# eBay/Sequence-Semantic-Embedding

Hardware: AMD Instinct MI355X
Metric: encoded seqs/sec (+ query x target cosine-scores/sec, top-1 vs ref) (higher is better)
Workload: dtype f32; 1 GPU; configs[1]: classification stand-in, dual-encoder LSTM H=S=256 E=50 T=32 V=32000; encode 16384 source seqs/GPU/step + cosine top-10 vs 571-target index; batch_per_gpu=16384, seq_len=32, targets=571, parallelism=dp1, weights=random-init (reference initialisers, seed 0)

## Files before the change

sequence-semantic-embedding_amd/csrc/score_topk.hip:

```cpp
#include <cstdlib>

#include "sse_kernels.h"

#define SC_THREADS 512
#define SC_KC 16
#ifndef SC_PRIO_K
#define SC_PRIO_K 1
#define SC_PRIO_E 0
#endif

#ifdef SSE_SCORE_CLOCK
#include <cstdio>
__device__ long long g_score_clk[8 * 8];
#define SC_CLK_DECL long long ck_[8] = {0, 0, 0, 0, 0, 0, 0, 0}, ck_t = clock64();
#define SC_CLK(i)                   \
  {                                 \
    const long long n_ = clock64(); \
    ck_[i] += n_ - ck_t;            \
    ck_t = n_;                      \
  }
#else
#define SC_CLK_DECL
#define SC_CLK(i)
#endif
// ... 671 lines not shown
                NQ, (int)BF, a.KG, w, v[w * 8 + 4], v[w * 8 + 0] / t, v[w * 8 + 1] / t, v[w * 8 + 2] / t, v[w * 8 + 5] / t, v[w * 8 + 6] / t, v[w * 8 + 7] / t,
                (v[w * 8 + 0] + v[w * 8 + 1] + v[w * 8 + 2] + v[w * 8 + 5] + v[w * 8 + 6]) / t);
      }
    }
  }
#endif
  return hipGetLastError();
}

template <int NQ, bool BF, bool COLLECT>
static hipError_t launch_score_variant(const ScoreArgs &a, hipStream_t stream) {
  return (a.KG % 8 == 0) ? launch_score_ringed<NQ, BF, COLLECT, true>(a, stream) : launch_score_ringed<NQ, BF, COLLECT, false>(a, stream);
}

__global__ void compact_uncert_kernel(const int32_t *cert, int Q, int32_t *qmap, int32_t *count) {
  const int q = blockIdx.x * blockDim.x + threadIdx.x;
  const bool open_q = q < Q && cert[q] == 0;
  const unsigned long long m = __ballot(open_q);
  if (m == 0ull) return;
  const int lane = threadIdx.x & 63;
  int base = 0;
  if (lane == __ffsll((long long)m) - 1) base = atomicAdd(count, __popcll(m));
  base = __shfl(base, __ffsll((long long)m) - 1);
  if (open_q) qmap[base + __popcll(m & ((1ull << lane) - 1ull))] = q;
}
__global__ void gather_query_rows_kernel(const float *q, const int32_t *qmap, const int32_t *count, int Q, int S, float *qc) {
  const int slot = blockIdx.x * (blockDim.x >> 6) + (threadIdx.x >> 6), lane = threadIdx.x & 63;
  const int n = *count, padded = min(Q, (n + 31) & ~31);
  if (slot >= padded) return;
  const float *src = slot < n ? q + (size_t)qmap[slot] * S : nullptr;
  for (int d = lane; d < S; d += 64) qc[(size_t)slot * S + d] = src ? src[d] : 0.0f;
}
hipError_t launch_compact_uncert(const float *q, const int32_t *cert, int Q, int S, int32_t *qmap, int32_t *count, float *qc,
                                 hipStream_t st) {
  hipError_t e = hipMemsetAsync(count, 0, sizeof(int32_t), st);
  if (e != hipSuccess) return e;
  hipLaunchKernelGGL(compact_uncert_kernel, dim3((Q + 255) / 256), dim3(256), 0, st, cert, Q, qmap, count);
  hipLaunchKernelGGL(gather_query_rows_kernel, dim3((Q + 3) / 4), dim3(256), 0, st, q, qmap, count, Q, S, qc);
  return hipGetLastError();
}

__global__ void count_uncert_kernel(const int32_t *cert, int Q, unsigned long long *count) {
  const int q = blockIdx.x * blockDim.x + threadIdx.x;
  const unsigned long long m = __ballot(q < Q && cert[q] == 0);
  if ((threadIdx.x & 63) == 0 && m) atomicAdd(count, (unsigned long long)__popcll(m));
}
hipError_t launch_count_uncert(const int32_t *cert, int Q, unsigned long long *count, hipStream_t st) {
  hipLaunchKernelGGL(count_uncert_kernel, dim3((Q + 255) / 256), dim3(256), 0, st, cert, Q, count);
  return hipGetLastError();
}

__global__ void pack_rows_bf16_kernel(const float *__restrict__ rows, int64_t R, int C, int KG16, int64_t total8,
                                      f32x4 *__restrict__ out) {
  for (int64_t i = (int64_t)blockIdx.x * blockDim.x + threadIdx.x; i < total8; i += (int64_t)gridDim.x * blockDim.x) {
    const int l = (int)(i & 63);
    const int64_t blk = i >> 6;
    const int kg = (int)(blk % KG16);
    const int64_t r = (blk / KG16) * 32 + (l & 31);
    const int k0 = kg * 16 + (l >> 5) * 8;
    unsigned w[4] = {0, 0, 0, 0};
    if (r < R) {
      const float *src = rows + (size_t)r * C + k0;
#pragma unroll
      for (int j = 0; j < 8; ++j) {
        unsigned short b = 0;
        if (k0 + j < C) {
          unsigned u = __float_as_uint(src[j]);
          u += 0x7FFFu + ((u >> 16) & 1u);
          b = (unsigned short)(u >> 16);
        }
        w[j >> 1] |= (unsigned)b << ((j & 1) * 16);
      }
    }
    out[i] = __builtin_bit_cast(f32x4, u32x4{w[0], w[1], w[2], w[3]});
  }
}

hipError_t launch_pack_rows_bf16(const float *rows, int64_t R, int C, void *out, hipStream_t stream) {
  const int KG16 = (C + 15) / 16;
  const int64_t total8 = ((R + 31) / 32) * KG16 * 64;
  if (total8 == 0) return hipSuccess;
  const int64_t blocks = (total8 + 255) / 256;
  hipLaunchKernelGGL(pack_rows_bf16_kernel, dim3((int)(blocks < 16384 ? blocks : 16384)), dim3(256), 0, stream, rows, R, C, KG16,
                     total8, reinterpret_cast<f32x4 *>(out));
  return hipGetLastError();
}

__global__ void frag32_to_bf16_kernel(const f32x4 *__restrict__ in, int64_t NT, int KG, int KG16, int64_t total8,
                                      f32x4 *__restrict__ out) {
  for (int64_t i = (int64_t)blockIdx.x * blockDim.x + threadIdx.x; i < total8; i += (int64_t)gridDim.x * blockDim.x) {
    const int l = (int)(i & 63);
    const int64_t blk = i >> 6;
    const int kg16 = (int)(blk % KG16);
    const int64_t tile = blk / KG16;
    const int kg = kg16 * 2 + (l >> 5), r = l & 31;
    f32x4 lo = {0, 0, 0, 0}, hi = {0, 0, 0, 0};
    if (kg < KG) {
      lo = in[((size_t)tile * KG + kg) * 64 + r];
      hi = in[((size_t)tile * KG + kg) * 64 + 32 + r];
    }
    unsigned w[4];
#pragma unroll
    for (int j = 0; j < 4; ++j) {
      const float a = (j < 2) ? lo[2 * j] : hi[2 * (j - 2)], b = (j < 2) ? lo[2 * j + 1] : hi[2 * (j - 2) + 1];
      unsigned ua = __float_as_uint(a), ub = __float_as_uint(b);
      ua += 0x7FFFu + ((ua >> 16) & 1u);
      ub += 0x7FFFu + ((ub >> 16) & 1u);
      w[j] = (ua >> 16) | (ub & 0xFFFF0000u);
    }
    out[i] = __builtin_bit_cast(f32x4, u32x4{w[0], w[1], w[2], w[3]});
  }
}

hipError_t launch_frag32_to_bf16(const float *idxp, int64_t NT, int KG, void *out, hipStream_t stream) {
  const int KG16 = (KG + 1) / 2;
  const int64_t total8 = NT * KG16 * 64;
  if (total8 == 0) return hipSuccess;
  const int64_t blocks = (total8 + 255) / 256;
  hipLaunchKernelGGL(frag32_to_bf16_kernel, dim3((int)(blocks < 16384 ? blocks : 16384)), dim3(256), 0, stream,
                     reinterpret_cast<const f32x4 *>(idxp), NT, KG, KG16, total8, reinterpret_cast<f32x4 *>(out));
  return hipGetLastError();
}

__global__ void frag32_to_split_bf16_kernel(const f32x4 *__restrict__ in, int KG, int KB, int64_t total8, sse_u32x4 *__restrict__ out) {
  for (int64_t i = (int64_t)blockIdx.x * blockDim.x + threadIdx.x; i < total8; i += (int64_t)gridDim.x * blockDim.x) {
    const int l = (int)(i & 63);
    const int64_t blk = i >> 6;
    const int kb = (int)(blk % KB);
    const int64_t tile = blk / KB;
    const int kg = kb * 2 + (l >> 5), r = l & 31;
    f32x4 lo4 = {0, 0, 0, 0}, hi4 = {0, 0, 0, 0};
    if (kg < KG) {
      lo4 = in[((size_t)tile * KG + kg) * 64 + r];
      hi4 = in[((size_t)tile * KG + kg) * 64 + 32 + r];
    }
    const float v[8] = {lo4[0], lo4[1], lo4[2], lo4[3], hi4[0], hi4[1], hi4[2], hi4[3]};
    sse_u32x4 h, lw;
    sse_split8(v, h, lw);
    out[(size_t)blk * 128 + l] = h;
    out[(size_t)blk * 128 + 64 + l] = lw;
  }
}

hipError_t launch_frag32_to_split_bf16(const float *idxp, int64_t NT, int KG, void *out, hipStream_t stream) {
  const int KB = (KG + 1) / 2;
  const int64_t total8 = NT * KB * 64;
  if (total8 == 0) return hipSuccess;
  const int64_t blocks = (total8 + 255) / 256;
  hipLaunchKernelGGL(frag32_to_split_bf16_kernel, dim3((int)(blocks < 16384 ? blocks : 16384)), dim3(256), 0, stream,
                     reinterpret_cast<const f32x4 *>(idxp), KG, KB, total8, reinterpret_cast<sse_u32x4 *>(out));
  return hipGetLastError();
}

__device__ __forceinline__ int si_key(float f) {
  const int i = __float_as_int(f);
  return i >= 0 ? i : (i ^ 0x7FFFFFFF);
}
__device__ __forceinline__ float si_val(int k) { return __int_as_float(k >= 0 ? k : (k ^ 0x7FFFFFFF)); }
template <int CTRL, int ROWMASK>
__device__ __forceinline__ float dpp_f(float x) {
  return __int_as_float(__builtin_amdgcn_update_dpp(__float_as_int(x), __float_as_int(x), CTRL, ROWMASK, 0xF, false));
}
__device__ __forceinline__ float wave_max_f(float x) {
  x = fmaxf(x, dpp_f<0x128, 0xF>(x));
  x = fmaxf(x, dpp_f<0x124, 0xF>(x));
  x = fmaxf(x, dpp_f<0x122, 0xF>(x));
  x = fmaxf(x, dpp_f<0x121, 0xF>(x));
  x = fmaxf(x, dpp_f<0x142, 0xA>(x));
  x = fmaxf(x, dpp_f<0x143, 0xC>(x));
  return __int_as_float(__builtin_amdgcn_readlane(__float_as_int(x), 63));
}
template <int JMAX>
#ifdef SSE_SCORE_CLOCK
#define SI_CLK_PARAMS , long long (&ck_)[8], long long &ck_t
#define SI_CLK_ARGS , ck_, ck_t
#else
#define SI_CLK_PARAMS
#define SI_CLK_ARGS
#endif
__device__ __forceinline__ void si_select4(const SmallIndexArgs &a, const float *sc, int NP, int NT, int qt, int q0, int lane SI_CLK_PARAMS) {
  constexpr int QW = 4;
  const int J = (NT * 32 + 63) / 64;
  float v[QW][JMAX];
#pragma unroll
  for (int j = 0; j < JMAX; ++j) {
    const int row = lane + 64 * j;
#pragma unroll
    for (int c = 0; c < QW; ++c) v[c][j] = (j < J && row < NT * 32) ? sc[(q0 + c) * NP + row] : NEG_INF;
  }
  int lok[QW], hik[QW];
  float lm[QW];
  bool done[QW];
#pragma unroll
  for (int c = 0; c < QW; ++c) {
    float m = NEG_INF;
#pragma unroll
    for (int j = 0; j < JMAX; ++j) m = fmaxf(m, v[c][j]);
    lm[c] = m;
    lok[c] = si_key(-wave_max_f(-m));
    hik[c] = si_key(wave_max_f(m)) + 1;
    done[c] = false;
  }
  SC_CLK(5)
  for (;;) {
    bool all_done = true;
#pragma unroll
    for (int c = 0; c < QW; ++c) {
      const unsigned width = (unsigned)hik[c] - (unsigned)lok[c];
      const int mid = lok[c] + (int)(width >> 1);
      const int cnt = __popcll(__ballot(lm[c] >= si_val(mid)));
      const bool open = !done[c] && width > 1u;
      const bool ge = cnt >= SC_KC;
      lok[c] = (open && ge) ? mid : lok[c];
      hik[c] = (open && !ge) ? mid : hik[c];
      done[c] = !open || (ge && cnt <= 24);
      all_done = all_done && done[c];
    }
    if (all_done) break;
  }
  SC_CLK(6)
#pragma unroll
  for (int c = 0; c < QW; ++c) {
    const int query = qt * 32 + q0 + c;
    if (query < a.Q) {
      const float T = si_val(lok[c]);
      float cs = NEG_INF;
      int cr = -1, base = 0;
#pragma unroll
      for (int j = 0; j < JMAX; ++j) {
        const bool take = (j < J) & (v[c][j] >= T) & (v[c][j] > NEG_INF);
        const unsigned long long mask = __ballot(take);
        const int n = __popcll(mask);
        const int slot = base + (int)__builtin_amdgcn_mbcnt_hi((unsigned)(mask >> 32), __builtin_amdgcn_mbcnt_lo((unsigned)mask, 0u));
        const int dst = (take && slot < 63) ? slot : 63;
        const int gs = __builtin_amdgcn_ds_permute(dst * 4, __float_as_int(v[c][j]));
        const int gr = __builtin_amdgcn_ds_permute(dst * 4, lane + 64 * j);
        const bool recv = (lane >= base) & (lane < base + n) & (lane < 63);
        cs = recv ? __int_as_float(gs) : cs;
        cr = recv ? gr : cr;
        base += n;
      }
      const int nw = base < 63 ? base : 63;
      int rank = 0;
      for (int l = 0; l < nw; ++l) {
        const float os = __int_as_float(__builtin_amdgcn_readlane(__float_as_int(cs), l));
        const int orow = __builtin_amdgcn_readlane(cr, l);
        rank += ((os > cs) | ((os == cs) & (orow < cr))) ? 1 : 0;
      }
      const bool mine = lane < nw;
      if (mine && rank < SC_KC) {
        a.part_scores[(size_t)query * SC_KC + rank] = cs;
        a.part_ids[(size_t)query * SC_KC + rank] = cr;
      }
      if (lane >= nw && lane < SC_KC) {
        a.part_scores[(size_t)query * SC_KC + lane] = NEG_INF;
        a.part_ids[(size_t)query * SC_KC + lane] = -1;
      }
      const unsigned long long m16 = __ballot(mine && rank == SC_KC - 1);
      const float last = m16 ? __int_as_float(__builtin_amdgcn_readlane(__float_as_int(cs), __ffsll((long long)m16) - 1)) : NEG_INF;
      if (lane == 0) a.part_bnd[query] = (base > 63) ? __builtin_inff() : last;
    }
  }
}

template <int KGC>
__global__ __launch_bounds__(256) void score_small_index_kernel(SmallIndexArgs a) {
  extern __shared__ __attribute__((aligned(16))) float si_sc[];
  const int tid = threadIdx.x, lane = tid & 63, w = __builtin_amdgcn_readfirstlane(tid >> 6);
  const int NT = a.NT, NP = NT * 32 + 1;
  const int qt = blockIdx.x;
  float *sc = si_sc;
  SC_CLK_DECL
  f32x4 b[KGC];
  {
    const int row = qt * 32 + (lane & 31), kb = (lane >> 5) * 4;
    const float *src = a.q_rows + (size_t)(row < a.Q ? row : 0) * a.S + kb;
    const bool vec = (a.S & 3) == 0 && (reinterpret_cast<uintptr_t>(a.q_rows) & 15) == 0 && KGC * 8 <= a.S;
#pragma unroll
    for (int kg = 0; kg < KGC; ++kg) {
      f32x4 v = {0, 0, 0, 0};
      if (vec) {
        v = *reinterpret_cast<const f32x4 *>(src + kg * 8);
      } else {
#pragma unroll
        for (int e = 0; e < 4; ++e)
          if (kg * 8 + kb + e < a.S) v[e] = src[kg * 8 + e];
      }
      if (row >= a.Q) v = f32x4{0, 0, 0, 0};
      b[kg] = v;
    }
  }
  SC_CLK(0)
  for (int t = w; t < NT; t += 4) {
    const f32x4 *ap = reinterpret_cast<const f32x4 *>(a.idxp) + (size_t)t * KGC * 64 + lane;
    f32x16 acc = {0, 0, 0, 0, 0, 0, 0, 0, 0, 0, 0, 0, 0, 0, 0, 0};
    f32x4 ar[4];
#pragma unroll
    for (int d = 0; d < 4; ++d) ar[d] = ap[(d < KGC ? d : 0) * 64];
#pragma unroll
    for (int kg = 0; kg < KGC; ++kg) {
      __builtin_amdgcn_sched_barrier(0);
#pragma unroll
      for (int e = 0; e < 4; ++e) acc = __builtin_amdgcn_mfma_f32_32x32x2f32(ar[kg & 3][e], b[kg][e], acc, 0, 0, 0);
      __builtin_amdgcn_sched_barrier(0);
      ar[kg & 3] = ap[(kg + 4 < KGC ? kg + 4 : kg) * 64];
    }
    const int rb = t * 32 + 4 * (lane >> 5);
    float *col = sc + (lane & 31) * NP;
#pragma unroll
    for (int r = 0; r < 16; ++r) {
      const int row = rb + (r & 3) + 8 * (r >> 2);
      col[row] = (row < a.N) ? acc[r] : NEG_INF;
    }
  }
  SC_CLK(1)
  __syncthreads();
  SC_CLK(2)
  if (NT * 32 <= 640) {
    si_select4<10>(a, sc, NP, NT, qt, w * 8, lane SI_CLK_ARGS);
    SC_CLK(3)
    si_select4<10>(a, sc, NP, NT, qt, w * 8 + 4, lane SI_CLK_ARGS);
    SC_CLK(4)
#ifdef SSE_SCORE_CLOCK
    if (blockIdx.x == gridDim.x / 2 && lane == 0)
      for (int i = 0; i < 8; ++i) g_score_clk[w * 8 + i] = ck_[i];
#endif
  } else {
    si_select4<16>(a, sc, NP, NT, qt, w * 8, lane SI_CLK_ARGS);
    si_select4<16>(a, sc, NP, NT, qt, w * 8 + 4, lane SI_CLK_ARGS);
  }
}
template <int KB>
__global__ __launch_bounds__(256) void score_small_index_x3_kernel(SmallIndexArgs a) {
  extern __shared__ __attribute__((aligned(16))) float si_sc[];
  const int tid = threadIdx.x, lane = tid & 63, w = __builtin_amdgcn_readfirstlane(tid >> 6);
  const int NT = a.NT, NP = NT * 32 + 1;
  const int qt = blockIdx.x;
  float *sc = si_sc;
  SC_CLK_DECL
  sse_u32x4 bh[KB], bl[KB];
  {
    const int row = qt * 32 + (lane & 31), kb0 = (lane >> 5) * 8;
    const float *src = a.q_rows + (size_t)(row < a.Q ? row : 0) * a.S + kb0;
    const bool vec = (a.S & 3) == 0 && (reinterpret_cast<uintptr_t>(a.q_rows) & 15) == 0 && KB * 16 <= a.S;
#pragma unroll
    for (int kb = 0; kb < KB; ++kb) {
      float v[8] = {0, 0, 0, 0, 0, 0, 0, 0};
      if (vec) {
        const f32x4 v0 = *reinterpret_cast<const f32x4 *>(src + kb * 16), v1 = *reinterpret_cast<const f32x4 *>(src + kb * 16 + 4);
#pragma unroll
        for (int e = 0; e < 4; ++e) {
          v[e] = v0[e];
          v[4 + e] = v1[e];
        }
      } else {
#pragma unroll
        for (int e = 0; e < 8; ++e)
          if (kb * 16 + kb0 + e < a.S) v[e] = src[kb * 16 + e];
      }
      if (row >= a.Q) {
#pragma unroll
        for (int e = 0; e < 8; ++e) v[e] = 0.0f;
      }
      sse_split8(v, bh[kb], bl[kb]);
    }
  }
  SC_CLK(0)
  {
    constexpr int D = KB < 4 ? KB : 4;
    static_assert(KB % D == 0, "the ring index must be static");
    const sse_u32x4 *img = reinterpret_cast<const sse_u32x4 *>(a.idx_x3) + lane;
    const sse_u32x4 *ap = img + (size_t)(w < NT ? w : 0) * KB * 128;
    sse_u32x4 ah[D], al[D];
#pragma unroll
    for (int d = 0; d < D; ++d) {
      ah[d] = ap[d * 128];
      al[d] = ap[d * 128 + 64];
    }
    for (int t = w; t < NT; t += 4) {
      const sse_u32x4 *apn = img + (size_t)(t + 4 < NT ? t + 4 : t) * KB * 128;
      f32x16 acc = {0, 0, 0, 0, 0, 0, 0, 0, 0, 0, 0, 0, 0, 0, 0, 0};
#pragma unroll
      for (int kb = 0; kb < KB; ++kb) {
        __builtin_amdgcn_sched_barrier(0);
        const bf16x8_t xh = __builtin_bit_cast(bf16x8_t, ah[kb % D]), xl = __builtin_bit_cast(bf16x8_t, al[kb % D]);
        const bf16x8_t yh = __builtin_bit_cast(bf16x8_t, bh[kb]), yl = __builtin_bit_cast(bf16x8_t, bl[kb]);
        acc = __builtin_amdgcn_mfma_f32_32x32x16_bf16(xh, yh, acc, 0, 0, 0);
        acc = __builtin_amdgcn_mfma_f32_32x32x16_bf16(xh, yl, acc, 0, 0, 0);
        acc = __builtin_amdgcn_mfma_f32_32x32x16_bf16(xl, yh, acc, 0, 0, 0);
        __builtin_amdgcn_sched_barrier(0);
        const sse_u32x4 *nx = (kb + D < KB) ? ap + (kb + D) * 128 : apn + (kb + D - KB) * 128;
        ah[kb % D] = nx[0];
        al[kb % D] = nx[64];
      }
      const int rb = t * 32 + 4 * (lane >> 5);
      float *col = sc + (lane & 31) * NP;
#pragma unroll
      for (int r = 0; r < 16; ++r) {
        const int row = rb + (r & 3) + 8 * (r >> 2);
        col[row] = (row < a.N) ? acc[r] : NEG_INF;
      }
      ap = apn;
    }
  }
  SC_CLK(1)
  __syncthreads();
  SC_CLK(2)
  if (NT * 32 <= 640) {
    si_select4<10>(a, sc, NP, NT, qt, w * 8, lane SI_CLK_ARGS);
    SC_CLK(3)
    si_select4<10>(a, sc, NP, NT, qt, w * 8 + 4, lane SI_CLK_ARGS);
    SC_CLK(4)
#ifdef SSE_SCORE_CLOCK
    if (blockIdx.x == gridDim.x / 2 && lane == 0)
      for (int i = 0; i < 8; ++i) g_score_clk[w * 8 + i] = ck_[i];
#endif
  } else {
    si_select4<16>(a, sc, NP, NT, qt, w * 8, lane SI_CLK_ARGS);
    si_select4<16>(a, sc, NP, NT, qt, w * 8 + 4, lane SI_CLK_ARGS);
  }
}
bool score_small_index_applies(int Q, int KG, int64_t NT) {
  return Q >= 1024 && (KG == 32 || KG == 8 || KG == 7) && NT * 32 <= 1024 && (size_t)32 * (NT * 32 + 1) * sizeof(float) <= (size_t)144 * 1024;
}
hipError_t launch_score_small_index(const SmallIndexArgs &a, hipStream_t stream) {
  if (!score_small_index_applies(a.Q, a.KG, a.NT)) return hipErrorInvalidValue;
  const size_t lds = (size_t)32 * (a.NT * 32 + 1) * sizeof(float);
  const dim3 grid((a.Q + 31) / 32), block(256);
  auto go = [&](auto kernel) -> hipError_t {
    hipError_t e = hipFuncSetAttribute(reinterpret_cast<const void *>(kernel), hipFuncAttributeMaxDynamicSharedMemorySize, (int)lds);
    if (e != hipSuccess) return e;
    hipLaunchKernelGGL(kernel, grid, block, lds, stream, a);
    return hipGetLastError();
  };
  if (a.idx_x3 && a.KG != 32) return go(score_small_index_x3_kernel<4>);
  if (a.KG == 8) return go(score_small_index_kernel<8>);
  if (a.KG == 7) return go(score_small_index_kernel<7>);
  const hipError_t e32 = a.idx_x3 ? go(score_small_index_x3_kernel<16>) : go(score_small_index_kernel<32>);
  if (e32 != hipSuccess) return e32;
#ifdef SSE_SCORE_CLOCK
  if (a.Q >= 8192) {
    static int n = 0;
    if (n++ % 8 == 3) {
      long long v[64];
      (void)hipStreamSynchronize(stream);
      (void)hipMemcpyFromSymbol(v, HIP_SYMBOL(g_score_clk), sizeof v);
      for (int w = 0; w < 4; w += 3)
        fprintf(stderr, "[small index clock Q=%d NT=%d] wave %d cycles: query fragments %lld | scores (MFMA + LDS stores) %lld | barrier %lld | selection: loads + bounds %lld | bisection %lld | winners + rank + stores %lld (both batches)\n",
                a.Q, a.NT, w, v[w * 8 + 0], v[w * 8 + 1], v[w * 8 + 2], v[w * 8 + 5], v[w * 8 + 6], v[w * 8 + 3] + v[w * 8 + 4]);
    }
  }
#endif
  return hipGetLastError();
}

hipError_t launch_score_topk(const ScoreArgs &a_in, hipStream_t stream) {
  ScoreArgs a = a_in;
#ifdef SSE_SCORE_MEASURE
  {
    static const int dbg = getenv("SSE_SCORE_DBG") ? atoi(getenv("SSE_SCORE_DBG")) : 0;
    a.dbg = dbg;
  }
#endif
  if (a.KC != SC_KC) return hipErrorInvalidValue;
  if (a.q_rows && ((a.NQ != 1 && !a.COLLECT) || a.S < 1)) return hipErrorInvalidValue;
  if (a.NSPLIT > 8 && (a.NSPLIT & 7)) return hipErrorInvalidValue;
  if (a.NSPLIT < 8 && (8 % a.NSPLIT)) return hipErrorInvalidValue;
  if (a.COLLECT) {
    if (!a.lane_max && (!a.col_thr || !a.col_slot || !a.col_cnt || !a.col_buf)) return hipErrorInvalidValue;
    if (a.BF) return a.NQ == 4 ? launch_score_variant<4, true, true>(a, stream) : hipErrorInvalidValue;
    if (a.NQ == 1) return launch_score_variant<1, false, true>(a, stream);
    if (a.NQ == 2) return launch_score_variant<2, false, true>(a, stream);
    if (a.NQ == 4) return launch_score_variant<4, false, true>(a, stream);
    return hipErrorInvalidValue;
  }
  if (!a.part_bnd) return hipErrorInvalidValue;
  if (a.BF) {
    if (a.NQ == 1) return launch_score_variant<1, true, false>(a, stream);
    if (a.NQ == 2) return launch_score_variant<2, true, false>(a, stream);
    if (a.NQ == 4) return launch_score_variant<4, true, false>(a, stream);
    return hipErrorInvalidValue;
  }
  if (a.NQ == 1) return launch_score_variant<1, false, false>(a, stream);
  if (a.NQ == 2) return launch_score_variant<2, false, false>(a, stream);
  if (a.NQ == 4) return launch_score_variant<4, false, false>(a, stream);
  return hipErrorInvalidValue;
}

template <int NB>
__device__ __forceinline__ void wave_exact_dot_n(const float *qrow, const float *idxp, const double *idx64, const int64_t (&n)[NB],
                                                 int S, int KG, int lane, double (&out)[NB]) {
  double acc[NB];
#pragma unroll
  for (int b = 0; b < NB; ++b) acc[b] = 0.0;
  if (idx64) {
    for (int d = lane; d < S; d += 64) {
      double rv[NB];
#pragma unroll
      for (int b = 0; b < NB; ++b) rv[b] = idx64[(size_t)n[b] * S + d];
#pragma unroll
      for (int b = 0; b < NB; ++b) acc[b] += (double)qrow[d] * rv[b];
    }
  } else {
    for (int j = lane; j < KG * 2; j += 64) {
      const int kg = j >> 1, half = j & 1;
      f32x4 v[NB];
#pragma unroll
      for (int b = 0; b < NB; ++b)
        v[b] = *reinterpret_cast<const f32x4 *>(idxp + (size_t)(n[b] >> 5) * KG * 256 + kg * 256 + (half * 32 + (int)(n[b] & 31)) * 4);
      const int d0 = kg * 8 + half * 4;
#pragma unroll
      for (int e = 0; e < 4; ++e)
        if (d0 + e < S) {
#pragma unroll
          for (int b = 0; b < NB; ++b) acc[b] += (double)qrow[d0 + e] * (double)v[b][e];
        }
    }
  }
#pragma unroll
  for (int o = 32; o > 0; o >>= 1)
#pragma unroll
    for (int b = 0; b < NB; ++b) acc[b] += __shfl_xor(acc[b], o);
#pragma unroll
  for (int b = 0; b < NB; ++b) out[b] = acc[b];
}
__device__ __forceinline__ double wave_exact_dot(const float *qrow, const float *idxp, const double *idx64,
                                                 int64_t n, int S, int KG, int lane) {
  const int64_t nn[1] = {n};
  double out[1];
  wave_exact_dot_n<1>(qrow, idxp, idx64, nn, S, KG, lane, out);
  return out[0];
}

template <int NB>
__device__ __forceinline__ int packed_value_of_lane(int lane) {
  int v = 0;
#pragma unroll
  for (int cnt = NB, bit = 5; cnt > 1; cnt >>= 1, --bit) v = v * 2 + ((lane >> bit) & 1);
  return v;
}
template <int NB>
__device__ __forceinline__ int packed_lane_of_value(int v) {
  int lane = 0;
#pragma unroll
  for (int cnt = NB, bit = 5; cnt > 1; cnt >>= 1, --bit) lane |= ((v / (cnt / 2)) & 1) << bit;
  return lane;
}
template <int NB>
__device__ __forceinline__ double wave_exact_dot_packed(const float *qrow, const float *idxp, const double *idx64, const int64_t (&n)[NB],
                                                        int S, int KG, int lane, const float *idx_rm = nullptr) {
  static_assert(NB == 2 || NB == 4 || NB == 8, "power of two");
  double acc[NB];
#pragma unroll
  for (int b = 0; b < NB; ++b) acc[b] = 0.0;
  if (idx64) {
    for (int d = lane; d < S; d += 64) {
      double rv[NB];
#pragma unroll
      for (int b = 0; b < NB; ++b) rv[b] = idx64[(size_t)n[b] * S + d];
#pragma unroll
      for (int b = 0; b < NB; ++b) acc[b] += (double)qrow[d] * rv[b];
    }
  } else {
    for (int j = lane; j < KG * 2; j += 64) {
      const int kg = j >> 1, half = j & 1;
      f32x4 v[NB];
#pragma unroll
      for (int b = 0; b < NB; ++b)
        v[b] = idx_rm ? *reinterpret_cast<const f32x4 *>(idx_rm + (size_t)n[b] * S + j * 4)
                      : *reinterpret_cast<const f32x4 *>(idxp + (size_t)(n[b] >> 5) * KG * 256 + kg * 256 + (half * 32 + (int)(n[b] & 31)) * 4);
      const int d0 = kg * 8 + half * 4;
#pragma unroll
      for (int e = 0; e < 4; ++e)
        if (d0 + e < S) {
#pragma unroll
          for (int b = 0; b < NB; ++b) acc[b] += (double)qrow[d0 + e] * (double)v[b][e];
        }
    }
  }
  int m = 32;
#pragma unroll
  for (int cnt = NB; cnt > 1; cnt >>= 1, m >>= 1) {
    const bool up = (lane & m) != 0;
#pragma unroll
    for (int i = 0; i < cnt / 2; ++i) {
      const double send = up ? acc[i] : acc[i + cnt / 2];
      const double keep = up ? acc[i + cnt / 2] : acc[i];
      acc[i] = keep + __shfl_xor(send, m);
    }
  }
#pragma unroll
  for (; m > 0; m >>= 1) acc[0] += __shfl_xor(acc[0], m);
  return acc[0];
}

__device__ __forceinline__ bool before(double sa, int64_t ia, double sb, int64_t ib) {
  return (sa > sb) || (sa == sb && ia < ib);
}

#define RS_THREADS 256
#define RS_MAXWIN 256
#define RS_MAXNC 4096
__global__ __launch_bounds__(RS_THREADS) void rescore_kernel(RescoreArgs a) {
  __shared__ int s_cnt;
  __shared__ int s_wid[RS_MAXWIN];
  __shared__ double s_ex[RS_MAXWIN];
  __shared__ float s_m[RS_THREADS / 64];
  __shared__ double s_qn[RS_THREADS / 64];
  extern __shared__ __attribute__((aligned(16))) unsigned long long s_key[];
  const int q = blockIdx.x, tid = threadIdx.x, lane = tid & 63, w = tid >> 6;
  if (a.uncert_clear && q == 0 && tid == 0) *a.uncert_clear = 0;
  if (a.q_count && q >= *a.q_count) return;
  const int qo = a.qmap ? a.qmap[q] : q;
  const float *ps = a.part_scores + (size_t)q * a.NC;
  const int32_t *pi = a.part_ids + (size_t)q * a.NC;
  const float *qrow = a.q + (size_t)q * a.S;
  const int KG = (a.S + 7) / 8;

  constexpr int PER = RS_MAXNC / RS_THREADS;
  float rs[PER];
  int ri[PER];
#pragma unroll
  for (int j = 0; j < PER; ++j) {
    const int c = tid + j * RS_THREADS;
    ri[j] = (c < a.NC) ? pi[c] : -1;
    rs[j] = (c < a.NC) ? ps[c] : NEG_INF;
  }
  float mmax = NEG_INF;
  for (int c = tid; c < a.NC / SC_KC; c += RS_THREADS) mmax = fmaxf(mmax, a.part_bnd[(size_t)q * (a.NC / SC_KC) + c]);

  {
    double v = 0.0;
    for (int d = tid; d < a.S; d += RS_THREADS) v += (double)qrow[d] * qrow[d];
#pragma unroll
    for (int o = 32; o > 0; o >>= 1) v += __shfl_xor(v, o);
    if (lane == 0) s_qn[w] = v;
  }
#pragma unroll
  for (int o = 32; o > 0; o >>= 1) mmax = fmaxf(mmax, __shfl_xor(mmax, o));
  if (lane == 0) s_m[w] = mmax;
  if (tid == 0) s_cnt = 0;

#pragma unroll
  for (int j = 0; j < PER; ++j) {
    const int c = tid + j * RS_THREADS;
    if (c < a.NC) {
      unsigned u = __float_as_uint(rs[j]);
      u = (u & 0x80000000u) ? ~u : (u | 0x80000000u);
      s_key[c] = (ri[j] < 0) ? 0ull : (((unsigned long long)u << 32) | (unsigned long long)(0xFFFFFFFFu - (unsigned)ri[j]));
    }
  }
  __syncthreads();
  const float qnorm = (float)sqrt(s_qn[0] + s_qn[1] + s_qn[2] + s_qn[3]);
  const float eps_q = a.eps * qnorm;
  mmax = fmaxf(fmaxf(s_m[0], s_m[1]), fmaxf(s_m[2], s_m[3]));
  float kth = NEG_INF;
  if (a.NC <= 256) {
    const unsigned long long key = (tid < a.NC) ? s_key[tid] : 0ull;
    int rank = 0;
    for (int j = 0; j < a.NC; ++j) rank += (s_key[j] > key) ? 1 : 0;
    float mine = (key != 0ull && rank == a.k - 1) ? rs[0] : NEG_INF;
#pragma unroll
    for (int o = 32; o > 0; o >>= 1) mine = fmaxf(mine, __shfl_xor(mine, o));
    __shared__ float s_thr[RS_THREADS / 64];
    if (lane == 0) s_thr[w] = mine;
    __syncthreads();
    kth = fmaxf(fmaxf(s_thr[0], s_thr[1]), fmaxf(s_thr[2], s_thr[3]));
  } else {
    __shared__ unsigned long long s_best[(RS_THREADS / 64) * SC_KC];
    const int nslots = a.NC / SC_KC;
    int head[RS_MAXNC / SC_KC / RS_THREADS];
#pragma unroll
    for (int j = 0; j < RS_MAXNC / SC_KC / RS_THREADS; ++j) head[j] = 0;
    for (int it = 0; it < a.k; ++it) {
      unsigned long long best = 0ull;
#pragma unroll
      for (int j = 0; j < RS_MAXNC / SC_KC / RS_THREADS; ++j) {
        const int slot = tid + j * RS_THREADS;
        if (slot < nslots && head[j] < SC_KC) {
          const unsigned long long key = s_key[slot * SC_KC + head[j]];
          best = key > best ? key : best;
        }
      }
      unsigned long long win = best;
#pragma unroll
      for (int o = 32; o > 0; o >>= 1) {
        const unsigned long long other = __shfl_xor(win, o);
        win = other > win ? other : win;
      }
      if (lane == 0) s_best[w * SC_KC + it] = win;
      if (win == 0ull) {
        for (int r = it + 1; r < a.k; ++r)
          if (lane == 0) s_best[w * SC_KC + r] = 0ull;
        break;
      }
#pragma unroll
      for (int j = 0; j < RS_MAXNC / SC_KC / RS_THREADS; ++j) {
        const int slot = tid + j * RS_THREADS;
        if (slot < nslots && head[j] < SC_KC && s_key[slot * SC_KC + head[j]] == win) ++head[j];
      }
    }
    __syncthreads();
    const int nk = (RS_THREADS / 64) * a.k;
    const unsigned long long key = (lane < nk) ? s_best[(lane / a.k) * SC_KC + lane % a.k] : 0ull;
    int rank = 0;
    for (int j = 0; j < nk; ++j) rank += (__shfl(key, j) > key) ? 1 : 0;
    unsigned long long kkey = (key != 0ull && rank == a.k - 1) ? key : 0ull;
#pragma unroll
    for (int o = 32; o > 0; o >>= 1) {
      const unsigned long long other = __shfl_xor(kkey, o);
      kkey = other > kkey ? other : kkey;
    }
    if (kkey != 0ull) {
      unsigned u = (unsigned)(kkey >> 32);
      u = (u & 0x80000000u) ? (u & 0x7FFFFFFFu) : ~u;
      kth = __uint_as_float(u);
    }
  }

#pragma unroll
  for (int j = 0; j < PER; ++j) {
    if (ri[j] >= 0 && rs[j] >= kth - 2.0f * eps_q) {
      const int p = atomicAdd(&s_cnt, 1);
      if (p < RS_MAXWIN) s_wid[p] = ri[j];
    }
  }
  __syncthreads();
  const int nwin_all = s_cnt;
  const int nwin = min(nwin_all, RS_MAXWIN);

  for (int i0 = w * 4; i0 < nwin; i0 += (RS_THREADS / 64) * 4) {
    int64_t n[4];
#pragma unroll
    for (int c = 0; c < 4; ++c) n[c] = s_wid[min(i0 + c, nwin - 1)];
    const double tot = wave_exact_dot_packed<4>(qrow, a.idx32, a.idx64, n, a.S, KG, lane, a.idx_rm);
    const int c = packed_value_of_lane<4>(lane);
    if ((lane & 15) == 0 && i0 + c < nwin) s_ex[i0 + c] = tot;
  }
  __syncthreads();

  double theta = -__builtin_inf();
  for (int i = tid; i < nwin; i += RS_THREADS) {
    const double s = s_ex[i];
    const int64_t id = s_wid[i];
    int rank = 0;
    for (int j = 0; j < nwin; ++j) rank += before(s_ex[j], (int64_t)s_wid[j], s, id);
    if (rank < a.k) {
      a.out_scores[(size_t)qo * a.k + rank] = s;
      a.out_ids[(size_t)qo * a.k + rank] = a.id_base + id;
      if (a.host_flag) {
        a.host_scores[(size_t)qo * a.k + rank] = s;
        a.host_ids[(size_t)qo * a.k + rank] = a.id_base + id;
      }
    }
    if (rank == a.k - 1) theta = s;
  }
  if (a.host_flag) __threadfence_system();
  {
    double t = theta;
#pragma unroll
    for (int o = 32; o > 0; o >>= 1) t = fmax(t, __shfl_xor(t, o));
    __syncthreads();
    if (lane == 0) s_ex[w] = t;
    __syncthreads();
    if (tid == 0) {
      t = fmax(fmax(s_ex[0], s_ex[1]), fmax(s_ex[2], s_ex[3]));
      const bool ok = (nwin_all <= RS_MAXWIN) && (nwin >= a.k) && ((double)mmax + (double)eps_q < t);
      a.cert[qo] = ok ? 1 : 0;
      if (!ok && a.uncert) atomicAdd(a.uncert, 1);
      if (a.col_thr) a.col_thr[qo] = ok ? __builtin_inff() : __double2float_rd(t - (double)(a.eps32 * qnorm));
      if (a.col_slot) {
        a.col_slot[qo] = ok ? -1 : qo;
        a.col_cnt[qo] = 0;
      }
      if (a.host_flag) {
        a.host_cert[qo] = ok ? 1 : 0;
        if (qo == 0 && a.host_err) *a.host_err = a.err_in ? *a.err_in : 0;
        __hip_atomic_store(a.host_flag + qo, a.seq, __ATOMIC_RELEASE, __HIP_MEMORY_SCOPE_SYSTEM);
      }
    }
  }
}

#ifndef RS_NB
#define RS_NB 4
#endif
__device__ __forceinline__ double readlane_f64(double v, int l) {
  const long long b = __double_as_longlong(v);
  const int lo = __builtin_amdgcn_readlane((int)b, l), hi = __builtin_amdgcn_readlane((int)(b >> 32), l);
  return __longlong_as_double(((long long)hi << 32) | (unsigned int)lo);
}
__global__ __launch_bounds__(256) void rescore_small_kernel(RescoreArgs a) {
  const int lane = threadIdx.x & 63;
  const int q = blockIdx.x * 4 + (threadIdx.x >> 6);
  if (a.uncert_clear && blockIdx.x == 0 && threadIdx.x == 0) *a.uncert_clear = 0;
  if (q >= a.Q) return;
  if (a.q_count && q >= *a.q_count) return;
  const int qo = a.qmap ? a.qmap[q] : q;
  const float *qrow = a.q + (size_t)q * a.S;
  const int KG = (a.S + 7) / 8;
#ifdef SSE_SCORE_CLOCK
  long long rk_[6] = {0, 0, 0, 0, 0, 0}, rk_t = clock64();
#define RS_CLK(i) { const long long n_ = clock64(); rk_[i] += n_ - rk_t; rk_t = n_; }
#else
#define RS_CLK(i)
#endif
  const bool have = lane < a.NC;
  const int id = have ? a.part_ids[(size_t)q * a.NC + lane] : -1;
  const float sc = have ? a.part_scores[(size_t)q * a.NC + lane] : NEG_INF;
  const float bnd = (lane < a.NC / SC_KC) ? a.part_bnd[(size_t)q * (a.NC / SC_KC) + lane] : NEG_INF;
  double qn = 0.0;
  for (int d = lane; d < a.S; d += 64) qn += (double)qrow[d] * qrow[d];
#pragma unroll
  for (int o = 32; o > 0; o >>= 1) qn += __shfl_xor(qn, o);
  const float qnorm = (float)sqrt(qn);
  const float eps_q = a.eps * qnorm;
  RS_CLK(0)

  unsigned u = __float_as_uint(sc);
  u = (u & 0x80000000u) ? ~u : (u | 0x80000000u);
  const unsigned long long key = (id < 0) ? 0ull : (((unsigned long long)u << 32) | (unsigned long long)(0xFFFFFFFFu - (unsigned)id));
  const int key_lo = (int)(unsigned)key, key_hi = (int)(unsigned)(key >> 32);
  int rank = 0;
  for (int j = 0; j < a.NC; ++j) {
    const unsigned long long kj = ((unsigned long long)(unsigned)__builtin_amdgcn_readlane(key_hi, j) << 32) |
                                  (unsigned long long)(unsigned)__builtin_amdgcn_readlane(key_lo, j);
    rank += (kj > key) ? 1 : 0;
  }
  const unsigned long long kmask = __ballot(key != 0ull && rank == a.k - 1);
  const float kth = kmask ? __int_as_float(__builtin_amdgcn_readlane(__float_as_int(sc), __ffsll((long long)kmask) - 1)) : NEG_INF;
  const bool in_win = (id >= 0) && (sc >= kth - 2.0f * eps_q);
  float mmax = NEG_INF;
  for (int j = 0; j < a.NC / SC_KC; ++j) mmax = fmaxf(mmax, __int_as_float(__builtin_amdgcn_readlane(__float_as_int(bnd), j)));
  const unsigned long long wmask = __ballot(in_win);
  const int nwin = __popcll(wmask);
  const int mi = __popcll(wmask & ((1ull << lane) - 1ull));
  const int idm = __builtin_amdgcn_ds_permute((in_win ? mi : 63) * 4, id);
  RS_CLK(1)
  double exm = -__builtin_inf();
  for (int m0 = 0; m0 < nwin; m0 += RS_NB) {
    int64_t n[RS_NB];
#pragma unroll
    for (int c = 0; c < RS_NB; ++c) n[c] = __builtin_amdgcn_readlane(idm, (m0 + c < nwin) ? m0 + c : 0);
    const double tot = wave_exact_dot_packed<RS_NB>(qrow, a.idx32, a.idx64, n, a.S, KG, lane, a.idx_rm);
    const int want = lane - m0;
    const double got = __shfl(tot, packed_lane_of_value<RS_NB>(want & (RS_NB - 1)));
    if (want >= 0 && want < RS_NB && lane < nwin) exm = got;
  }
  RS_CLK(2)
  int r2 = 0;
  for (int j = 0; j < nwin; ++j)
    r2 += before(readlane_f64(exm, j), (int64_t)__builtin_amdgcn_readlane(idm, j), exm, (int64_t)idm) ? 1 : 0;
  const bool member = lane < nwin;
  if (member && r2 < a.k) {
    a.out_scores[(size_t)qo * a.k + r2] = exm;
    a.out_ids[(size_t)qo * a.k + r2] = a.id_base + idm;
    if (a.host_flag) {
      a.host_scores[(size_t)qo * a.k + r2] = exm;
      a.host_ids[(size_t)qo * a.k + r2] = a.id_base + idm;
    }
  }
  const unsigned long long tmask = __ballot(member && r2 == a.k - 1);
  const double theta = tmask ? readlane_f64(exm, __ffsll((long long)tmask) - 1) : -__builtin_inf();
  if (a.host_flag) __threadfence_system();
  RS_CLK(3)
#ifdef SSE_SCORE_CLOCK
  if (q == a.Q / 2 && lane == 0) {
    rk_[4] = nwin;
    for (int i = 0; i < 6; ++i) g_score_clk[i] = rk_[i];
  }
#endif
  if (lane == 0) {
    const bool ok = (nwin >= a.k) && ((double)mmax + (double)eps_q < theta);
    a.cert[qo] = ok ? 1 : 0;
    if (!ok && a.uncert) atomicAdd(a.uncert, 1);
    if (a.col_thr) a.col_thr[qo] = ok ? __builtin_inff() : __double2float_rd(theta - (double)(a.eps32 * qnorm));
    if (a.col_slot) {
      a.col_slot[qo] = ok ? -1 : qo;
      a.col_cnt[qo] = 0;
    }
    if (a.host_flag) {
      a.host_cert[qo] = ok ? 1 : 0;
      if (qo == 0 && a.host_err) *a.host_err = a.err_in ? *a.err_in : 0;
      __hip_atomic_store(a.host_flag + qo, a.seq, __ATOMIC_RELEASE, __HIP_MEMORY_SCOPE_SYSTEM);
    }
  }
}

hipError_t launch_rescore(const RescoreArgs &a, hipStream_t stream) {
  if (a.NC > RS_MAXNC) return hipErrorInvalidValue;
  if (a.NC <= 64) {
    hipLaunchKernelGGL(rescore_small_kernel, dim3((a.Q + 3) / 4), dim3(256), 0, stream, a);
#ifdef SSE_SCORE_CLOCK
    if (a.Q >= 8192) {
      static int n = 0;
      if (n++ % 8 == 3) {
        long long v[8];
        (void)hipStreamSynchronize(stream);
        (void)hipMemcpyFromSymbol(v, HIP_SYMBOL(g_score_clk), sizeof v);
        fprintf(stderr, "[rescore_small clock Q=%d NC=%d] cycles: query norm %lld | candidates, rank, k-th, window %lld | float64 dots %lld (window of %lld) | exact rank + outputs %lld\n",
                a.Q, a.NC, v[0], v[1], v[2], v[4], v[3]);
      }
    }
#endif
    return hipGetLastError();
  }
  hipLaunchKernelGGL(rescore_kernel, dim3(a.Q), dim3(RS_THREADS), (size_t)a.NC * sizeof(unsigned long long), stream, a);
  return hipGetLastError();
}

#define EX_THREADS 256
struct ExactArgs {
  const float *q;
  const float *idxp;
  const double *idx64;
  const int32_t *cert;
  double *out_scores;
  int64_t *out_ids;
  int64_t id_base, N;
  int32_t Q, S, k;
  int32_t k_off, k_total;
  unsigned long long *served;
  const int32_t *uncert;
};

__device__ __forceinline__ void exact_topk_query(const ExactArgs a, const int q, double (*s_sc)[SC_KC],
                                                 int64_t (*s_id)[SC_KC]) {
  const int tid = threadIdx.x, lane = tid & 63, w = tid >> 6;
  if (a.served && tid == 0 && a.k_off == 0) atomicAdd(a.served, 1ull);
  const float *qrow = a.q + (size_t)q * a.S;
  const int KG = (a.S + 7) / 8;
  double ls[SC_KC];
  int64_t li[SC_KC];
#pragma unroll
  for (int i = 0; i < SC_KC; ++i) {
    ls[i] = -__builtin_inf();
    li[i] = -1;
  }
  double cut_s = __builtin_inf();
  int64_t cut_id = -1;
  if (a.k_off > 0) {
    cut_s = a.out_scores[(size_t)q * a.k_total + a.k_off - 1];
    cut_id = a.out_ids[(size_t)q * a.k_total + a.k_off - 1] - a.id_base;
  }
  for (int64_t n = w; n < a.N; n += EX_THREADS / 64) {
    double s = wave_exact_dot(qrow, a.idxp, a.idx64, n, a.S, KG, lane);
    const bool after_cut = (s < cut_s) || (s == cut_s && n > cut_id);
    if (after_cut && s > ls[SC_KC - 1]) {
      int64_t id = n;
      bool ins = false;
#pragma unroll
      for (int i = 0; i < SC_KC; ++i) {
        const bool gt = ins || (s > ls[i]);
        ins = gt;
        const double tv = ls[i];
        const int64_t ti = li[i];
        ls[i] = gt ? s : tv;
        li[i] = gt ? id : ti;
        s = gt ? tv : s;
        id = gt ? ti : id;
      }
    }
  }
  if (lane == 0) {
#pragma unroll
    for (int i = 0; i < SC_KC; ++i) {
      s_sc[w][i] = ls[i];
      s_id[w][i] = li[i];
    }
  }
  __syncthreads();
  if (tid == 0) {
    unsigned pos4 = 0;
    auto pos = [&](int p) { return (int)((pos4 >> (8 * p)) & 0xFFu); };
    for (int o = 0; o < a.k; ++o) {
      int best = -1;
      for (int p = 0; p < EX_THREADS / 64; ++p) {
        if (pos(p) >= SC_KC || s_id[p][pos(p)] < 0) continue;
        if (best < 0 || before(s_sc[p][pos(p)], s_id[p][pos(p)], s_sc[best][pos(best)], s_id[best][pos(best)])) best = p;
      }
      a.out_scores[(size_t)q * a.k_total + a.k_off + o] = s_sc[best][pos(best)];
      a.out_ids[(size_t)q * a.k_total + a.k_off + o] = a.id_base + s_id[best][pos(best)];
      pos4 += 1u << (8 * best);
    }
  }
}
__global__ __launch_bounds__(EX_THREADS) void exact_topk_kernel(ExactArgs a) {
  __shared__ double s_sc[EX_THREADS / 64][SC_KC];
  __shared__ int64_t s_id[EX_THREADS / 64][SC_KC];
  const int q = blockIdx.x;
  if (a.cert && a.cert[q]) return;
  exact_topk_query(a, q, s_sc, s_id);
}
__global__ __launch_bounds__(EX_THREADS) void exact_topk_strided_kernel(ExactArgs a) {
  __shared__ double s_sc[EX_THREADS / 64][SC_KC];
  __shared__ int64_t s_id[EX_THREADS / 64][SC_KC];
  __shared__ unsigned char s_open[EX_THREADS];
  if (a.uncert && *a.uncert == 0) return;
  {
    const long long q = (long long)blockIdx.x + (long long)threadIdx.x * gridDim.x;
    s_open[threadIdx.x] = (q < a.Q) && !(a.cert && a.cert[q]);
  }
  __syncthreads();
  int it = 0;
#pragma nounroll
  for (int q = blockIdx.x; q < a.Q; q += gridDim.x, ++it) {
    const bool open = it < EX_THREADS ? s_open[it] != 0 : !(a.cert && a.cert[q]);
    if (!open) continue;
    exact_topk_query(a, q, s_sc, s_id);
    __syncthreads();
  }
}

hipError_t launch_exact_topk(const float *q, const float *idxp, const double *idx64, const int32_t *cert,
                             double *out_scores, int64_t *out_ids, int64_t id_base, int64_t N, int Q, int S,
                             int k, hipStream_t stream, unsigned long long *served, const int32_t *uncert, int grid_cap) {
  for (int off = 0; off < k; off += SC_KC) {
    ExactArgs a{q, idxp, idx64, cert, out_scores, out_ids, id_base, N, Q, S, (k - off < SC_KC) ? k - off : SC_KC, off, k, served, uncert};
    const int grid = (uncert && grid_cap > 0 && grid_cap < Q) ? grid_cap : Q;
    if (grid < Q) hipLaunchKernelGGL(exact_topk_strided_kernel, dim3(grid), dim3(EX_THREADS), 0, stream, a);
    else hipLaunchKernelGGL(exact_topk_kernel, dim3(Q), dim3(EX_THREADS), 0, stream, a);
  }
  return hipGetLastError();
}


__global__ void assign_slots_kernel(const int32_t *cert, int Q, int slots, int32_t *col_slot, int32_t *counter) {
  const int q = blockIdx.x * blockDim.x + threadIdx.x;
  if (q >= Q) return;
  int slot = -1;
  if (cert[q] == 0) {
    slot = atomicAdd(counter, 1);
    if (slot >= slots) slot = -1;
  }
  col_slot[q] = slot;
}
hipError_t launch_assign_slots(const int32_t *cert, int Q, int slots, int32_t *col_slot, int32_t *counter, hipStream_t st) {
  hipLaunchKernelGGL(assign_slots_kernel, dim3((Q + 255) / 256), dim3(256), 0, st, cert, Q, slots, col_slot, counter);
  return hipGetLastError();
}

__device__ __forceinline__ void lds_sort_desc_u64(unsigned long long *key, int n2, int tid, int nthr) {
  for (int size = 2; size <= n2; size <<= 1)
    for (int stride = size >> 1; stride > 0; stride >>= 1) {
      __syncthreads();
      for (int i = tid; i < (n2 >> 1); i += nthr) {
        const int lo = 2 * i - (i & (stride - 1)), hi = lo + stride;
        const bool desc = ((lo & size) == 0);
        const unsigned long long x = key[lo], y = key[hi];
        if ((x < y) == desc) {
          key[lo] = y;
          key[hi] = x;
        }
      }
    }
  __syncthreads();
}

__global__ __launch_bounds__(256) void kth_bound_kernel(const float *q, const float *part_scores, const int32_t *part_ids, int Q,
                                                        int S, int NC, int k, float eps, float *col_thr, int32_t *col_slot) {
// ... 198 lines not shown
```

sequence-semantic-embedding_amd/csrc/sse_api.hip:

```cpp
#include <cmath>
#include <cstdarg>
#include <cstdio>
#include <cstdlib>
#include <algorithm>
#include <chrono>
#include <cstring>
#include <dlfcn.h>
#include <link.h>
#include <mutex>
#include <string>
#include <vector>

#include "../../include/sse_hip.h"
#include "sse_kernels.h"
#include "train.h"

namespace {

thread_local std::string g_create_error;

struct Variable {
  std::string name;
  int rows = 0, cols = 0;
  int64_t count = 0;
  float *dev = nullptr;
  float *slot = nullptr;
  float *grad = nullptr;
};

struct PadTable {
  float *h = nullptr, *c = nullptr;
  int T = 0, cap = 0;
  bool valid = false;
  void release() {
    if (h) (void)hipFree(h);
    if (c) (void)hipFree(c);
    h = c = nullptr;
  }
};

struct Encoder {
  int kernel = -1, bias = -1, proj = -1;
  int H = 0, Hp = 0, UB = 0, KGx = 0, KGh = 0, Ep = 0;
  float *Wp = nullptr, *Mp = nullptr;
  float *Waug = nullptr;
  bool waug_valid = false;
  float *Wc = nullptr;
  bool wc_valid = false;
  unsigned short *Wx3 = nullptr;
  bool x3_valid = false;
  unsigned short *Wx3t = nullptr;
  int shares_lstm_with = -1;
  bool generic = false;
  PadTable pad_fwd, pad_small, pad_x3;
  float *xtab = nullptr;
  bool xtab_valid = false;
};

struct DevBuf {
  void *p = nullptr;
  size_t cap = 0;
  DevBuf() = default;
  DevBuf(const DevBuf &) = delete;
  DevBuf &operator=(const DevBuf &) = delete;
  ~DevBuf() {
    if (p) (void)hipFree(p);
  }
};

struct TrainState {
  DevBuf ids[2], labels, raw[2], draw[2], tape_g[2], tape_a[2], h_last[2], dh_last[2], dg_a[2], dg_b[2], db_part[2],
      dk_part[2], dm_part[2], sq_part, norm_part, row_loss, row_acc, scal;
  DevBuf feat_rm, pos, dfeat, dw_part, dbias_part, wt, wct;
  uint64_t gen_ver[2] = {0, 0};
  DevBuf gen_A[2], gen_tape[2], gen_dG[2], gen_hl[2], gen_KT[2], gen_Kq[2], gen_MT[2], gen_G, gen_c, gen_dA, gen_dc, gen_dkp;
  hipStream_t side[2] = {nullptr, nullptr};
  hipEvent_t ev_fork = nullptr, ev_join[2] = {nullptr, nullptr};
  float *KhT[2] = {nullptr, nullptr}, *KxT[2] = {nullptr, nullptr};
  unsigned short *KhT16[2] = {nullptr, nullptr};
  unsigned short *KxT16[2] = {nullptr, nullptr};
  bool packed_dirty = true;
  bool fp32_dirty = true;
  float *arena = nullptr;
  bool arena_external = false, grads_ready = false;
  DevBuf corpus[2], rows[2];
  int64_t corpus_N[2] = {0, 0};
  int32_t corpus_T[2] = {0, 0};
  bool rows_mode = false;
  bool defer_err = false;
  DevBuf ids_raw[2], perm, hot_part[2];
  int perm_B = 0;
  std::vector<int32_t> h_perm, h_rows[2], h_tgt;
  std::vector<float> h_labels;
};

}

enum { PATH_PERSIST, PATH_CLUSTER, PATH_SMALL, PATH_X3, PATH_GENERIC, PATH_FWD, PATH_FWD_ROWS32, PATH_FWD_ROWS64, PATH_FWD_GS, PATH_FWD_XT,
       PATH_COUNT };
static const char *const LSTM_PATH_NAMES[PATH_COUNT] = {"lstm_path_persist", "lstm_path_cluster", "lstm_path_small", "lstm_path_x3",
                                                "lstm_path_generic", "lstm_path_fwd", "lstm_fwd_rows32", "lstm_fwd_rows64",
                                                "lstm_fwd_gate_split", "lstm_fwd_x_table"};

struct sse_handle {
  sse_config cfg;
  std::mutex mu;
  std::string err;
  std::vector<Variable> vars;
  Encoder enc[2];
  bool packed_dirty = true;
  uint64_t weights_version = 1;
  bool mp_fresh = false;
  bool pad_skip = true;
  int pad_sort_dev = 1;
  int64_t score_two_pass_min_rows = 49152, score_two_pass_rows = 524288;
  int64_t two_pass_calls = 0;
  DevBuf s_lmax;
  bool lstm_gate_split = true;
  DevBuf s_padzero, s_padwork, s_padorder;
  int32_t *pad_stat = nullptr;
  int32_t pad_seq = 0;
  int64_t pad_sorted_calls = 0;
  int64_t lstm_path_calls[10] = {0, 0, 0, 0, 0, 0, 0, 0, 0, 0};
  bool lstm_x3 = false;
  unsigned short *emb16 = nullptr;
  bool emb16_valid = false;
  int lstm_persist_rows = 32;
  uint32_t persist_epoch = 0;
  hipStream_t stream = nullptr;
  bool persist_inject = false;
  int64_t persist_fallbacks = 0;
  int cu_count = 0;
  int lstm_cluster_rows = 1024;
  uint32_t cluster_epoch = 0;
  int lstm_cluster_chunks = 3;
  int cluster_backoff = -1;
  int cluster_skip[2] = {0, 0};
  int lstm_cluster_coop = 1;
  int lstm_cluster_wt = 0;
  int lstm_cluster_drop = 0;
  int lstm_small_rows = 1024;
  int lstm_x_table = 1;
  int lstm_x_table_mb = 256;
  int64_t x_table_builds = 0;
  bool score_small_index = true;
  bool score_small_x3 = true;
  bool score_bf16 = true;
  void *idxp16 = nullptr;
  size_t idxp16_cap = 0;
  bool idxp16_valid = false;
  bool fb_cnt_init = false;
  int uncert_word = 0;
  bool cnn_bf16 = false;
  unsigned short *emb_bf16 = nullptr, *cnn_Wc16 = nullptr, *cnn_Mx3 = nullptr;
  int lstm_train_rows = 0;
  bool train_bwd_x3 = false;
  bool train_fwd_x3 = false;
  bool train_dk_x3 = false;
  bool train_generic = false;
  bool train_gen1 = false;
  bool train_pair_dedup = true;
  bool train_serial = false;
  float *emb_pad = nullptr;
  int cnn_W[4] = {-1, -1, -1, -1}, cnn_b[4] = {-1, -1, -1, -1}, cnn_M = -1, tgt_table = -1;
  float *cnn_Wc = nullptr, *cnn_bias = nullptr, *cnn_Mp = nullptr;
  int32_t *err_flag = nullptr;
  float *idxp = nullptr;
  size_t idxp_cap = 0;
  double *idx64 = nullptr;
  DevBuf idx_rm;
  bool idx_rm_valid = false;
  DevBuf idx_x3;
  bool idx_x3_valid = false;
  int64_t idx_N = 0, idx_base = 0;
  int idx_S = 0;
  float idx_norm_max = 1.0f;
  DevBuf s_ids, s_out, s_q, s_qp, s_ps, s_pi, s_cert, s_os, s_oi, s_tmp, s_tmp2, s_feat, s_zero, s_map;
  DevBuf s_qmap, s_qc;
  DevBuf s_qp32, s_fb_cnt;
  DevBuf g_A, g_G, g_c, g_hl, g_raw;
  DevBuf g_KT[2], g_Kq[2], g_MT[2];
  uint64_t g_ver[2] = {0, 0};
  DevBuf s_xchg;
  DevBuf s_persist;
  DevBuf s_cluster;
  int32_t *pin_small = nullptr;
  void *pin = nullptr;
  size_t pin_cap = 0;
  int32_t score_seq = 0;
  DevBuf s_pb, s_cthr, s_cslot, s_ccnt, s_cbuf;
  int eval_chunk_rows = 65536;
  int64_t eval_paired_calls = 0;
  DevBuf ev_ids[2], ev_stage, ev_rows[2], ev_labels, ev_raw[2], ev_row, ev_sums;
  float lr = 0.9f;
  int64_t global_step = 0;
  TrainState *train = nullptr;
  std::vector<hipEvent_t> events;
};

namespace {

int fail(sse_handle *h, const char *fmt, ...) {
  char buf[512];
  va_list ap;
  va_start(ap, fmt);
  vsnprintf(buf, sizeof buf, fmt, ap);
  va_end(ap);
  if (h) h->err = buf; else g_create_error = buf;
  return 1;
}

#define HIPCHECK(h, expr)                                                                         \
  do {                                                                                            \
    hipError_t e_ = (expr);                                                                       \
    if (e_ != hipSuccess) return fail(h, "%s failed: %s (%s:%d)", #expr, hipGetErrorString(e_), __FILE__, __LINE__); \
  } while (0)

hipError_t sync_stream(hipStream_t st) {
  const auto t0 = std::chrono::steady_clock::now();
  for (;;) {
    const hipError_t e = hipStreamQuery(st);
    if (e != hipErrorNotReady) return e;
    if (std::chrono::steady_clock::now() - t0 > std::chrono::milliseconds(3)) return hipStreamSynchronize(st);
  }
}

int reserve(sse_handle *h, DevBuf &b, size_t bytes) {
  if (bytes <= b.cap) return 0;
  if (b.p) HIPCHECK(h, hipFree(b.p));
  b.p = nullptr;
  b.cap = 0;
  const size_t cap = bytes + bytes / 4 + 256;
  HIPCHECK(h, hipMalloc(&b.p, cap));
  b.cap = cap;
  return 0;
}

int add_var(sse_handle *h, const std::string &name, int rows, int cols) {
  Variable v;
  v.name = name;
  v.rows = rows;
  v.cols = cols;
  v.count = (int64_t)rows * cols;
  h->vars.push_back(v);
  return (int)h->vars.size() - 1;
}

int find_var(sse_handle *h, const char *name, bool *is_slot) {
  std::string n(name);
  *is_slot = false;
  const std::string suffix = "/Adagrad";
  if (n.size() > suffix.size() && n.compare(n.size() - suffix.size(), suffix.size(), suffix) == 0) {
    n.resize(n.size() - suffix.size());
    *is_slot = true;
  }
  for (size_t i = 0; i < h->vars.size(); ++i)
    if (h->vars[i].name == n) return (int)i;
  return -1;
}

int setup_encoder(sse_handle *h, Encoder &e, const std::string &scope, const std::string &proj, int H, int proj_rows) {
  const sse_config &c = h->cfg;
  e.H = H;
  e.kernel = add_var(h, scope + "/rnn/basic_lstm_cell/kernel", c.embedding_size + H, 4 * H);
  e.bias = add_var(h, scope + "/rnn/basic_lstm_cell/bias", 1, 4 * H);
  e.proj = add_var(h, proj, proj_rows, c.encoding_size);
  return 0;
}

int geometry(sse_handle *h, Encoder &e) {
  const sse_config &c = h->cfg;
  if (e.H <= 0) return 0;
  e.Hp = e.H <= 128 ? 128 : e.H <= 256 ? 256 : round_up(e.H, 512);
  e.UB = e.Hp / 128;
  e.Ep = round_up(c.embedding_size + 1, 8);
  e.KGx = e.Ep / 8;
  e.KGh = e.Hp / 8;
  e.generic = e.H > 512 || c.encoding_size > 512 || lstm_fwd_lds_bytes(e.KGx, e.KGh, e.Hp == 512 ? 1 : 2) > 160 * 1024;
  return 0;
}

static int emb_cols(const sse_config &c) {
  return c.network_mode == SSE_MODE_SOURCE_ONLY_CNN ? round_up(c.embedding_size, 4) : round_up(c.embedding_size + 1, 8);
}

Encoder &lstm_owner(sse_handle *h, Encoder &e) { return e.shares_lstm_with >= 0 ? h->enc[e.shares_lstm_with] : e; }

void invalidate_derived(Encoder &e) {
  e.waug_valid = e.wc_valid = e.x3_valid = false;
  e.pad_fwd.valid = e.pad_small.valid = e.pad_x3.valid = false;
  e.xtab_valid = false;
}

int ensure_proj_packed(sse_handle *h, hipStream_t st) {
  if (!h->packed_dirty || h->mp_fresh) return 0;
  const sse_config &c = h->cfg;
  for (int s = 0; s < 2; ++s) {
    Encoder &e = h->enc[s];
// ... 740 lines not shown
                   out_s + (size_t)q0 * k, out_i + (size_t)q0 * k, (int32_t *)h->s_cert.p, h->idx_base, Qc, S, k, counters + 1};
    HIPCHECK(h, launch_select_topk(sel, st));
    HIPCHECK(h, launch_exact_topk(qc, h->idxp, h->idx64, (const int32_t *)h->s_cert.p, out_s + (size_t)q0 * k,
                                  out_i + (size_t)q0 * k, h->idx_base, h->idx_N, Qc, S, k, st, counters + 2));
  }
  return 0;
}

enum { SCORE_ALL = 0, SCORE_FIRST = 1, SCORE_REST = 2 };
struct ScoreMirror {
  double *scores;
  int64_t *ids;
  int32_t *cert, *err, *flag;
  int32_t seq;
};
int score_dev_locked(sse_handle *h, const float *q, int Q, int k, double *out_s, int64_t *out_i, hipStream_t st,
                     int phase = SCORE_ALL, int *split = nullptr, const ScoreMirror *mirror = nullptr) {
  if (split) *split = 0;
  if (!h->idxp) return fail(h, "no index uploaded");
  if (Q < 0) return fail(h, "bad Q");
  if (Q == 0) return 0;
  if (k < 1 || k > h->idx_N) return fail(h, "k=%d must be in [1, N=%lld]", k, (long long)h->idx_N);
  if ((k > 16) && phase == SCORE_REST) return 0;
  if (k > SSE_MAX_SELECT_K) {
    HIPCHECK(h, launch_exact_topk(q, h->idxp, h->idx64, nullptr, out_s, out_i, h->idx_base, h->idx_N, Q, h->idx_S, k, st));
    return 0;
  }
  if (k > 16) return score_select_locked(h, q, Q, k, out_s, out_i, st);
  const int S = h->idx_S, KG = (S + 7) / 8;
  const int QT = (Q + 31) / 32;
  const bool bf = h->score_bf16 && h->idx_N >= 8192;
  const int NQ = score_pick_nq(Q, S, bf ? 1 : 0);
  if (NQ == 0) return fail(h, "index dimension %d does not fit the scoring kernel's LDS query block", S);
  const int QB = (QT + NQ - 1) / NQ;
  const int64_t NT = (h->idx_N + 31) / 32;
  const int nsplit = choose_nsplit(NQ, QB, NT);
  int nsplit2 = nsplit;
  static const int split2_max = getenv("SSE_SPLIT2_MAX") ? atoi(getenv("SSE_SPLIT2_MAX")) : 128;
  while (nsplit2 < split2_max && NT / (nsplit2 * 2 * 2) >= 16) nsplit2 *= 2;
  const bool small_idx = h->score_small_index && !bf && score_small_index_applies(Q, KG, NT);
  const bool small_x3 = small_idx && h->score_small_x3 && h->idx_x3_valid;
  const int NC = small_idx ? 16 : nsplit * 16, NCmax = std::max(nsplit, nsplit2) * 16;
  const int KG16 = (S + 15) / 16;
  if (bf && !h->idxp16_valid) {
    const size_t need = (size_t)NT * KG16 * 1024;
    if (need > h->idxp16_cap) {
      if (h->idxp16) HIPCHECK(h, hipFree(h->idxp16));
      h->idxp16 = nullptr;
      h->idxp16_cap = 0;
      HIPCHECK(h, hipMalloc(&h->idxp16, need));
      h->idxp16_cap = need;
    }
    HIPCHECK(h, launch_frag32_to_bf16(h->idxp, NT, KG, h->idxp16, st));
    h->idxp16_valid = true;
  }
  if (ensure_counters(h, st)) return 1;
  unsigned long long *counters = (unsigned long long *)h->s_fb_cnt.p;
  if (bf && NQ == 4 && Q >= 1024 && h->idx_N >= h->score_two_pass_min_rows && h->idx_N <= h->score_two_pass_rows && !mirror) {
    int ns2 = std::min(nsplit, 16);
    {
      static const int force = getenv("SSE_TWO_PASS_SPLITS") ? atoi(getenv("SSE_TWO_PASS_SPLITS")) : 0;
      const int cus = h->cu_count > 0 ? h->cu_count : 256;
      double best = 0.0;
      for (int ns = 1; ns <= 16; ns *= 2) {
        if (ns > 1 && NT / ns < 32) break;
        const double r = (double)QB * ns / cus, eff = r / std::ceil(r);
        if (eff > best + 0.02) {
          best = eff;
          ns2 = ns;
        }
      }
      if (force == 1 || force == 2 || force == 4 || force == 8 || force == 16) ns2 = force;
    }
    if (phase == SCORE_REST) return 0;
    h->two_pass_calls += 1;
    constexpr int MID_CAP = 512;
    const float eps32 = (float)(2.0 * (S + 2) * 5.97e-8 * h->idx_norm_max);
    const float eps_bf = eps32 + (float)(1.02 * (1.0 / 256.0 + 1.0 / 262144.0) * h->idx_norm_max);
    if (reserve(h, h->s_qp, (size_t)QB * NQ * KG * 256 * sizeof(float))) return 1;
    if (reserve(h, h->s_lmax, (size_t)Q * ns2 * 16 * sizeof(float))) return 1;
    if (reserve(h, h->s_cert, (size_t)Q * sizeof(int32_t))) return 1;
    if (reserve(h, h->s_cthr, (size_t)Q * sizeof(float)) || reserve(h, h->s_cslot, (size_t)Q * sizeof(int32_t)) ||
        reserve(h, h->s_ccnt, (size_t)(Q + 1) * sizeof(int32_t)) || reserve(h, h->s_cbuf, (size_t)Q * MID_CAP * sizeof(int32_t)))
      return 1;
    HIPCHECK(h, launch_pack_rows_bf16(q, Q, S, h->s_qp.p, st));
    HIPCHECK(h, hipMemsetAsync(h->s_ccnt.p, 0, (size_t)(Q + 1) * sizeof(int32_t), st));
    HIPCHECK(h, hipMemsetAsync(h->s_cert.p, 0, (size_t)Q * sizeof(int32_t), st));
    ScoreArgs m1;
    m1.BF = 1;
    m1.COLLECT = 1;
    m1.idxp = (const float *)h->idxp16;
    m1.qp = (const float *)h->s_qp.p;
    m1.N = h->idx_N;
    m1.Q = Q;
    m1.KG = KG16;
    m1.NT = (int)NT;
    m1.QT = QT;
    m1.NSPLIT = ns2;
    m1.KC = 16;
    m1.NQ = NQ;
    m1.lane_max = (float *)h->s_lmax.p;
    HIPCHECK(h, launch_score_topk(m1, st));
    HIPCHECK(h, launch_lane_max_threshold(q, (const float *)h->s_lmax.p, Q, S, ns2 * 16, eps_bf, (float *)h->s_cthr.p,
                                          (int32_t *)h->s_cslot.p, st));
    ScoreArgs m2 = m1;
    m2.lane_max = nullptr;
    m2.col_thr = (const float *)h->s_cthr.p;
    m2.col_slot = (const int32_t *)h->s_cslot.p;
    m2.col_cnt = (int32_t *)h->s_ccnt.p;
    m2.col_buf = (int32_t *)h->s_cbuf.p;
    m2.col_cap = MID_CAP;
    HIPCHECK(h, launch_score_topk(m2, st));
    SelectArgs sel{q, h->idxp, h->idx64, m2.col_slot, m2.col_cnt, m2.col_buf, MID_CAP, out_s, out_i, (int32_t *)h->s_cert.p, h->idx_base,
                   Q, S, k, nullptr};
    HIPCHECK(h, launch_select_topk(sel, st));
    HIPCHECK(h, launch_exact_topk(q, h->idxp, h->idx64, (const int32_t *)h->s_cert.p, out_s, out_i, h->idx_base, h->idx_N, Q, S, k, st,
                                  counters + 2));
    if (split) *split = 0;
    return 0;
  }
  const int POOL = std::min(Q, 1024);
  if (reserve(h, h->s_qp, (size_t)QB * NQ * KG * 256 * sizeof(float))) return 1;
  if (reserve(h, h->s_ps, (size_t)Q * (bf ? NCmax : NC) * sizeof(float))) return 1;
  if (reserve(h, h->s_pi, (size_t)Q * (bf ? NCmax : NC) * sizeof(int32_t))) return 1;
  if (reserve(h, h->s_pb, (size_t)Q * (bf ? NCmax / 16 : nsplit) * sizeof(float))) return 1;
  if (reserve(h, h->s_cert, (size_t)Q * sizeof(int32_t))) return 1;
  if (reserve_collect(h, Q, POOL)) return 1;
  if (split) *split = 1;
  const bool first = phase != SCORE_REST, rest = phase != SCORE_FIRST;
  const bool rows_direct = NQ == 1;
  if (first && !rows_direct && !small_idx) {
    if (bf) HIPCHECK(h, launch_pack_rows_bf16(q, Q, S, h->s_qp.p, st));
    else HIPCHECK(h, launch_pack_rows(q, Q, S, (float *)h->s_qp.p, st));
  }
  ScoreArgs a;
  if (rows_direct) {
    a.q_rows = q;
    a.S = S;
  }
  a.BF = bf ? 1 : 0;
  a.idxp = bf ? (const float *)h->idxp16 : h->idxp;
  a.qp = (const float *)h->s_qp.p;
  a.part_scores = (float *)h->s_ps.p;
  a.part_ids = (int32_t *)h->s_pi.p;
  a.part_bnd = (float *)h->s_pb.p;
  a.N = h->idx_N;
  a.Q = Q;
  a.KG = bf ? KG16 : KG;
  a.NT = (int)NT;
  a.QT = QT;
  a.NSPLIT = nsplit;
  a.KC = 16;
  a.NQ = NQ;
  if (first) {
    if (small_idx) {
      SmallIndexArgs si{q, h->idxp, a.part_scores, a.part_ids, a.part_bnd, h->idx_N, Q, S, KG, (int)NT};
      if (small_x3) si.idx_x3 = h->idx_x3.p;
      HIPCHECK(h, launch_score_small_index(si, st));
    } else {
      HIPCHECK(h, launch_score_topk(a, st));
    }
  }
  RescoreArgs r;
  r.q = q;
  r.idx32 = h->idxp;
  r.idx64 = h->idx64;
  r.idx_rm = h->idx_rm_valid ? (const float *)h->idx_rm.p : nullptr;
  r.part_scores = a.part_scores;
  r.part_ids = a.part_ids;
  r.part_bnd = a.part_bnd;
  r.out_scores = out_s;
  r.out_ids = out_i;
  r.cert = (int32_t *)h->s_cert.p;
  r.id_base = h->idx_base;
  r.N = h->idx_N;
  r.Q = Q;
  r.S = S;
  r.NC = NC;
  r.k = k;
  const float eps32 = (float)(2.0 * (S + 2) * 5.97e-8 * h->idx_norm_max);
  r.eps = eps32;
  r.eps32 = eps32;
  r.col_thr = (float *)h->s_cthr.p;
  if (first) h->uncert_word ^= 1;
  int32_t *const uncert = (int32_t *)(counters + 4) + h->uncert_word;
  const int follow_grid = 2 * (h->cu_count > 0 ? h->cu_count : 256);
  r.uncert = uncert;
  r.uncert_clear = (int32_t *)(counters + 4) + (h->uncert_word ^ 1);
  const bool own_slots = Q <= POOL;
  if (own_slots) {
    r.col_slot = (int32_t *)h->s_cslot.p;
    r.col_cnt = (int32_t *)h->s_ccnt.p;
  }
  if (bf) r.eps += (float)(1.02 * (1.0 / 256.0 + 1.0 / 262144.0) * h->idx_norm_max);
  if (small_x3)
    r.eps = (float)(((1.0 + 1.0 / 64.0) / 32768.0 + 2.0 * (3 * S + 2) * 5.97e-8 * (1.0 + 1.0 / 32.0)) * h->idx_norm_max);
  if (first) {
    RescoreArgs rf = r;
    if (mirror) {
      rf.host_scores = mirror->scores;
      rf.host_ids = mirror->ids;
      rf.host_cert = mirror->cert;
      rf.host_err = mirror->err;
      rf.host_flag = mirror->flag;
      rf.err_in = h->err_flag;
      rf.seq = mirror->seq;
    }
    HIPCHECK(h, launch_rescore(rf, st));
  }
  if (!rest) return 0;
  const float *qp32 = (const float *)h->s_qp.p;
  if (bf && Q > 32) {
    if (reserve(h, h->s_qp32, (size_t)QB * NQ * KG * 256 * sizeof(float))) return 1;
    if (reserve(h, h->s_qmap, (size_t)(Q + 1) * sizeof(int32_t))) return 1;
    if (reserve(h, h->s_qc, (size_t)QT * 32 * S * sizeof(float))) return 1;
    HIPCHECK(h, launch_count_uncert(r.cert, Q, counters, st));
    int32_t *qmap = (int32_t *)h->s_qmap.p, *qcount = qmap + Q;
    HIPCHECK(h, launch_compact_uncert(q, r.cert, Q, S, qmap, qcount, (float *)h->s_qc.p, st));
    if (!rows_direct) HIPCHECK(h, launch_pack_rows((const float *)h->s_qc.p, Q, S, (float *)h->s_qp32.p, st));
    ScoreArgs a2 = a;
    a2.BF = 0;
    a2.idxp = h->idxp;
    a2.qp = (const float *)h->s_qp32.p;
    if (rows_direct) a2.q_rows = (const float *)h->s_qc.p;
    a2.KG = KG;
    a2.q_count = qcount;
    a2.NSPLIT = nsplit2;
    HIPCHECK(h, launch_score_topk(a2, st));
    RescoreArgs r2 = r;
    r2.q = (const float *)h->s_qc.p;
    r2.NC = nsplit2 * 16;
    r2.eps = eps32;
    r2.qmap = qmap;
    r2.q_count = qcount;
    r2.uncert = r2.uncert_clear = nullptr;
    HIPCHECK(h, launch_rescore(r2, st));
    qp32 = (const float *)h->s_qp32.p;
  }
  if (!own_slots) {
    HIPCHECK(h, hipMemsetAsync(h->s_ccnt.p, 0, (size_t)(POOL + 1) * sizeof(int32_t), st));
    HIPCHECK(h, launch_assign_slots(r.cert, Q, POOL, (int32_t *)h->s_cslot.p, (int32_t *)h->s_ccnt.p + POOL, st));
  }
  ScoreArgs c = a;
  c.BF = 0;
  c.idxp = h->idxp;
  c.qp = qp32;
  c.q_rows = q;
  c.S = S;
  c.KG = KG;
  c.COLLECT = 1;
  c.col_thr = (const float *)h->s_cthr.p;
  c.col_slot = (const int32_t *)h->s_cslot.p;
  c.col_cnt = (int32_t *)h->s_ccnt.p;
  c.col_buf = (int32_t *)h->s_cbuf.p;
  c.col_cap = SSE_COLLECT_CAP;
  c.uncert = uncert;
  HIPCHECK(h, launch_score_topk(c, st));
  SelectArgs sel{q, h->idxp, h->idx64, c.col_slot, c.col_cnt, c.col_buf, SSE_COLLECT_CAP, out_s, out_i, r.cert, h->idx_base, Q, S, k,
                 counters + 1, uncert, follow_grid};
  HIPCHECK(h, launch_select_topk(sel, st));
  HIPCHECK(h, launch_exact_topk(q, h->idxp, h->idx64, r.cert, out_s, out_i, h->idx_base, h->idx_N, Q, S, k, st, counters + 2, uncert,
                                follow_grid));
  return 0;
}

}

extern "C" {

const char *sse_last_error(sse_handle *h) { return h ? h->err.c_str() : g_create_error.c_str(); }

int sse_create(const sse_config *cfg, sse_handle **out) {
  if (!cfg || !out) return fail(nullptr, "sse_create: null argument");
  *out = nullptr;
  int ndev = 0;
  if (hipGetDeviceCount(&ndev) != hipSuccess || ndev == 0) return fail(nullptr, "no HIP device available");
  if (cfg->device < 0 || cfg->device >= ndev) return fail(nullptr, "device %d out of range (have %d)", cfg->device, ndev);
  if (cfg->vocab_size < 2 || cfg->embedding_size < 1 || cfg->encoding_size < 1)
    return fail(nullptr, "bad model sizes V=%d E=%d S=%d", cfg->vocab_size, cfg->embedding_size, cfg->encoding_size);
  sse_handle *h = new sse_handle();
  h->cfg = *cfg;
  h->lr = cfg->learning_rate;
#define CREATE_FAIL(...)        \
  do {                          \
    fail(nullptr, __VA_ARGS__); \
    sse_destroy(h);             \
    return 1;                   \
  } while (0)
  if (hipSetDevice(cfg->device) != hipSuccess) CREATE_FAIL("hipSetDevice(%d) failed", cfg->device);
  add_var(h, "word_embedding", cfg->vocab_size, cfg->embedding_size);
  switch (cfg->network_mode) {
    case SSE_MODE_DUAL_ENCODER:
      setup_encoder(h, h->enc[0], "source_encoder", "source_encoder/src_M", cfg->src_cell_size, cfg->src_cell_size);
      setup_encoder(h, h->enc[1], "target_encoder", "target_encoder/tgt_M", cfg->tgt_cell_size, cfg->tgt_cell_size);
      break;
    case SSE_MODE_SHARED_ENCODER:
      setup_encoder(h, h->enc[0], "shared_encoder", "shared_encoder/src_M", cfg->src_cell_size, cfg->src_cell_size);
      h->enc[1] = h->enc[0];
      h->enc[1].proj = add_var(h, "shared_encoder/tgt_M", cfg->src_cell_size, cfg->encoding_size);
      h->enc[1].shares_lstm_with = 0;
      break;
    case SSE_MODE_SOURCE_ENCODER_ONLY:
      setup_encoder(h, h->enc[0], "source_only_encoder", "source_only_encoder/src_M", cfg->src_cell_size, cfg->src_cell_size);
      h->tgt_table = add_var(h, "target_embedding/tgt_seq_embedding", cfg->target_space_size, cfg->encoding_size);
      break;
    case SSE_MODE_SOURCE_ONLY_CNN: {
      static const int fs[4] = {2, 3, 4, 5}, nf[4] = {256, 128, 128, 64};
      for (int i = 0; i < 4; ++i) {
        char nm[96];
        snprintf(nm, sizeof nm, "source_only_cnn/conv-maxpool-%d/W", fs[i]);
        h->cnn_W[i] = add_var(h, nm, fs[i] * cfg->embedding_size, nf[i]);
        snprintf(nm, sizeof nm, "source_only_cnn/conv-maxpool-%d/b", fs[i]);
        h->cnn_b[i] = add_var(h, nm, 1, nf[i]);
      }
      h->cnn_M = add_var(h, "source_only_cnn/src_M", 576, cfg->encoding_size);
      h->tgt_table = add_var(h, "target_embedding/tgt_seq_embedding", cfg->target_space_size, cfg->encoding_size);
      break;
    }
    default:
      CREATE_FAIL("Unsupported network mode %d (sse_model.py:175-177)", cfg->network_mode);
  }
  for (int s = 0; s < 2; ++s)
    if (h->enc[s].kernel >= 0 && geometry(h, h->enc[s])) {
      g_create_error = h->err;
      sse_destroy(h);
      return 1;
    }
  for (auto &v : h->vars) {
    if (hipMalloc((void **)&v.dev, v.count * sizeof(float)) != hipSuccess ||
        hipMalloc((void **)&v.slot, v.count * sizeof(float)) != hipSuccess)
      CREATE_FAIL("hipMalloc failed for variable %s", v.name.c_str());
    hipMemset(v.dev, 0, v.count * sizeof(float));
    launch_fill(v.slot, v.count, 0.1f, nullptr);
  }
  if (hipMalloc((void **)&h->err_flag, sizeof(int32_t)) != hipSuccess) CREATE_FAIL("hipMalloc failed");
  if (hipHostMalloc((void **)&h->pin_small, 64 * sizeof(int32_t), hipHostMallocDefault) != hipSuccess) CREATE_FAIL("hipHostMalloc failed");
  hipMemset(h->err_flag, 0, sizeof(int32_t));
  if (hipHostMalloc((void **)&h->pad_stat, 8 * sizeof(int32_t), hipHostMallocDefault) != hipSuccess) CREATE_FAIL("hipHostMalloc failed");
  {
    hipDeviceProp_t prop;
    if (hipGetDeviceProperties(&prop, cfg->device) == hipSuccess) h->cu_count = prop.multiProcessorCount;
  }
  if (const char *ev = getenv("SSE_PAD_SORT_DEV")) {
    const int v = atoi(ev);
    if (v >= 0 && v <= 2) h->pad_sort_dev = v;
  }
  memset(h->pad_stat, 0, 8 * sizeof(int32_t));
  if (hipDeviceSynchronize() != hipSuccess) CREATE_FAIL("device initialisation failed");
#undef CREATE_FAIL
  *out = h;
// ... 201 lines not shown
  return 0;
}

static int score_to_host_locked(sse_handle *h, const float *q_dev, int Q, int k, double *out_scores, int64_t *out_ids,
                                int32_t *err_bits = nullptr) {
  hipStream_t st = nullptr;
  if (reserve(h, h->s_os, (size_t)Q * k * sizeof(double))) return 1;
  if (reserve(h, h->s_oi, (size_t)Q * k * sizeof(int64_t))) return 1;
  const size_t nb = (size_t)Q * k * 8, need = 2 * nb + (size_t)(2 * Q + 1) * sizeof(int32_t);
  if (ensure_pin(h, need)) return 1;
  char *pin = (char *)h->pin;
  int32_t *cert = (int32_t *)(pin + 2 * nb), *flag = cert + Q, *done = flag + 1;
  int split = 0;
  const bool use_mirror = Q <= 64 && k <= 16;
  ScoreMirror hm{(double *)pin, (int64_t *)(pin + nb), cert, flag, done, 0};
  if (use_mirror) {
    h->score_seq = (h->score_seq == INT32_MAX) ? 1 : h->score_seq + 1;
    hm.seq = h->score_seq;
    for (int i = 0; i < Q; ++i) __atomic_store_n(done + i, 0, __ATOMIC_RELAXED);
    __atomic_store_n(flag, 0, __ATOMIC_RELEASE);
  }
  if (score_dev_locked(h, q_dev, Q, k, (double *)h->s_os.p, (int64_t *)h->s_oi.p, st, SCORE_FIRST, &split, use_mirror ? &hm : nullptr))
    return 1;
  int pass = 0;
  if (use_mirror && split) {
    const auto t0 = std::chrono::steady_clock::now();
    bool synced = false;
    for (;;) {
      bool all = true;
      for (int i = 0; i < Q && all; ++i) all = __atomic_load_n(done + i, __ATOMIC_ACQUIRE) == hm.seq;
      if (all) break;
      if (synced) return fail(h, "the re-scoring pass did not report completion");
      if (std::chrono::steady_clock::now() - t0 > std::chrono::milliseconds(3)) {
        HIPCHECK(h, hipStreamSynchronize(st));
        synced = true;
      }
    }
    if (err_bits) {
      *err_bits = *flag;
      if (*flag) return 0;
    }
    bool open_q = false;
    for (int i = 0; i < Q && !open_q; ++i) open_q = cert[i] == 0;
    if (open_q) {
      if (score_dev_locked(h, q_dev, Q, k, (double *)h->s_os.p, (int64_t *)h->s_oi.p, st, SCORE_REST)) return 1;
      pass = 1;
    } else {
      pass = 2;
    }
  }
  for (; pass < 2; ++pass) {
    HIPCHECK(h, hipMemcpyAsync(pin, h->s_os.p, nb, hipMemcpyDeviceToHost, st));
    HIPCHECK(h, hipMemcpyAsync(pin + nb, h->s_oi.p, nb, hipMemcpyDeviceToHost, st));
    if (split && pass == 0) HIPCHECK(h, hipMemcpyAsync(cert, h->s_cert.p, (size_t)Q * sizeof(int32_t), hipMemcpyDeviceToHost, st));
    if (err_bits && pass == 0) HIPCHECK(h, hipMemcpyAsync(flag, h->err_flag, sizeof(int32_t), hipMemcpyDeviceToHost, st));
    HIPCHECK(h, sync_stream(st));
    if (err_bits && pass == 0) {
      *err_bits = *flag;
      if (*flag) return 0;
    }
    bool open_q = false;
    if (split && pass == 0) {
      for (int i = 0; i < Q && !open_q; ++i) open_q = cert[i] == 0;
    }
    if (!open_q) break;
    if (score_dev_locked(h, q_dev, Q, k, (double *)h->s_os.p, (int64_t *)h->s_oi.p, st, SCORE_REST)) return 1;
  }
  memcpy(out_scores, pin, nb);
  memcpy(out_ids, pin + nb, nb);
  return 0;
}

int sse_encode_score_topk(sse_handle *h, int side, const int32_t *ids_host, int32_t B, int32_t T, int32_t normalize,
                          int32_t k, double *out_scores, int64_t *out_ids, float *enc_out_host) {
  if (!h) return 1;
  std::lock_guard<std::mutex> lk(h->mu);
  HIPCHECK(h, hipSetDevice(h->cfg.device));
  if (B == 0) return 0;
  if (B < 0 || T < 1 || !ids_host || !out_scores || !out_ids) return fail(h, "bad arguments to sse_encode_score_topk");
  if (!h->idxp) return fail(h, "no index uploaded");
  if (h->cfg.encoding_size != h->idx_S)
    return fail(h, "index dimension %d != encoding_size %d", h->idx_S, h->cfg.encoding_size);
  if (encode_host_ids_locked(h, side, ids_host, B, T, normalize, true)) return 1;
  int32_t bits = 0;
  if (score_to_host_locked(h, (const float *)h->s_out.p, B, k, out_scores, out_ids, &bits)) return 1;
  if (bits) {
    if (check_err_flag(h, nullptr, &bits)) return 1;
    if (bits == 4) {
      if (encode_fallback_locked(h, side, B, T, normalize, nullptr)) return 1;
      if (score_to_host_locked(h, (const float *)h->s_out.p, B, k, out_scores, out_ids)) return 1;
    }
  }
  if (enc_out_host)
    HIPCHECK(h, hipMemcpy(enc_out_host, h->s_out.p, (size_t)B * h->cfg.encoding_size * sizeof(float), hipMemcpyDeviceToHost));
  return 0;
}

int sse_get_counter(sse_handle *h, const char *name, int64_t *value) {
  if (!h || !name || !value) return 1;
  std::lock_guard<std::mutex> lk(h->mu);
  if (strcmp(name, "lstm_persist_fallbacks") == 0) {
    *value = h->persist_fallbacks;
    return 0;
  }
  if (strcmp(name, "score_two_pass_calls") == 0) {
    *value = h->two_pass_calls;
    return 0;
  }
  if (strcmp(name, "pad_sorted_calls") == 0) {
    *value = h->pad_sorted_calls;
    return 0;
  }
  if (strcmp(name, "eval_paired_calls") == 0) {
    *value = h->eval_paired_calls;
    return 0;
  }
  if (strcmp(name, "lstm_x_table_builds") == 0) {
    *value = h->x_table_builds;
    return 0;
  }
  for (int i = 0; i < PATH_COUNT; ++i) {
    if (strcmp(name, LSTM_PATH_NAMES[i]) != 0) continue;
    *value = h->lstm_path_calls[i];
    return 0;
  }
  if (strcmp(name, "lstm_coop_refused") == 0) {
    *value = (int64_t)lstm_coop_refused();
    return 0;
  }
  static const char *const names[3] = {"score_bf16_second_chance_queries", "score_collect_queries", "score_bruteforce_queries"};
  for (int i = 0; i < 3; ++i) {
    if (strcmp(name, names[i]) != 0) continue;
    unsigned long long v[4] = {0, 0, 0, 0};
    if (h->s_fb_cnt.p && h->fb_cnt_init) {
      HIPCHECK(h, hipSetDevice(h->cfg.device));
      HIPCHECK(h, hipDeviceSynchronize());
      HIPCHECK(h, hipMemcpy(v, h->s_fb_cnt.p, sizeof v, hipMemcpyDeviceToHost));
    }
    *value = (int64_t)v[i];
    return 0;
  }
  return fail(h, "unknown counter '%s'", name);
}

int sse_set_option(sse_handle *h, const char *name, int32_t value) {
  if (!h || !name) return 1;
  std::lock_guard<std::mutex> lk(h->mu);
  if (strcmp(name, "score_small_index") == 0) {
    h->score_small_index = value != 0;
    return 0;
  }
  if (strcmp(name, "score_small_x3") == 0) {
    h->score_small_x3 = value != 0;
    return 0;
  }
  if (strcmp(name, "score_bf16") == 0) {
    h->score_bf16 = value != 0;
    return 0;
  }
  if (strcmp(name, "cnn_bf16") == 0) {
    if (h->cfg.network_mode != SSE_MODE_SOURCE_ONLY_CNN) return fail(h, "option cnn_bf16 needs network_mode source_only_cnn");
    h->cnn_bf16 = value != 0;
    h->packed_dirty = true;
    h->mp_fresh = false;
    return 0;
  }
  if (strcmp(name, "lstm_train_rows") == 0) {
    if (value != 0 && value != 32 && value != 64) return fail(h, "lstm_train_rows must be 0, 32 or 64");
    h->lstm_train_rows = (int)value;
    return 0;
  }
  if (strcmp(name, "train_bwd_x3") == 0) {
    h->train_bwd_x3 = value != 0;
    return 0;
  }
  if (strcmp(name, "train_fwd_x3") == 0) {
    h->train_fwd_x3 = value != 0;
    return 0;
  }
  if (strcmp(name, "train_dk_x3") == 0) {
    h->train_dk_x3 = value != 0;
    return 0;
  }
  if (strcmp(name, "train_generic") == 0) {
    h->train_generic = value != 0;
    return 0;
  }
  if (strcmp(name, "train_gen1") == 0) {
    h->train_gen1 = value != 0;
    return 0;
  }
  if (strcmp(name, "train_pair_dedup") == 0) {
    h->train_pair_dedup = value != 0;
    return 0;
  }
  if (strcmp(name, "eval_chunk_rows") == 0) {
    if (value < 2) return fail(h, "eval_chunk_rows must be >= 2");
    h->eval_chunk_rows = (int)(value & ~1);
    return 0;
  }
  if (strcmp(name, "train_serial") == 0) {
    h->train_serial = value != 0;
    return 0;
  }
  if (strcmp(name, "pad_skip") == 0) {
    h->pad_skip = value != 0;
    return 0;
  }
  if (strcmp(name, "score_two_pass_min_rows") == 0) {
    if (value < 0) return fail(h, "score_two_pass_min_rows must be >= 0");
    h->score_two_pass_min_rows = value;
    return 0;
  }
  if (strcmp(name, "score_two_pass_rows") == 0) {
    if (value < 0) return fail(h, "score_two_pass_rows must be >= 0");
    h->score_two_pass_rows = value;
    return 0;
  }
  if (strcmp(name, "lstm_gate_split") == 0) {
    h->lstm_gate_split = value != 0;
    return 0;
  }
  if (strcmp(name, "pad_sort_dev") == 0) {
    if (value < 0 || value > 2) return fail(h, "pad_sort_dev must be 0 (off), 1 (adaptive) or 2 (always)");
    h->pad_sort_dev = (int)value;
    return 0;
  }
  if (strcmp(name, "lstm_x3") == 0) {
    h->lstm_x3 = value != 0;
    return 0;
  }
  if (strcmp(name, "lstm_persist_epoch") == 0) {
    if (value < 0 || value >= (1 << 20)) return fail(h, "lstm_persist_epoch must be in [0, 2^20)");
    h->persist_epoch = (uint32_t)value;
    return 0;
  }
  if (strcmp(name, "lstm_persist_inject_miss") == 0) {
    h->persist_inject = value != 0;
    return 0;
  }
  if (strcmp(name, "lstm_persist_rows") == 0) {
    if (value < 0) return fail(h, "lstm_persist_rows must be >= 0");
    h->lstm_persist_rows = (int)value;
    return 0;
  }
  if (strcmp(name, "lstm_cluster_backoff") == 0) {
    if (value < -1) return fail(h, "lstm_cluster_backoff must be >= 0 (or -1: automatic)");
    h->cluster_backoff = (int)value;
    h->cluster_skip[0] = h->cluster_skip[1] = 0;
    return 0;
  }
  if (strcmp(name, "lstm_cluster_chunks") == 0) {
    if (value < 1) return fail(h, "lstm_cluster_chunks must be >= 1");
    h->lstm_cluster_chunks = (int)value;
    return 0;
  }
  if (strcmp(name, "lstm_cluster_drop_wg") == 0) {
    h->lstm_cluster_drop = value != 0;
    return 0;
  }
  if (strcmp(name, "lstm_cluster_coop") == 0) {
    h->lstm_cluster_coop = value != 0;
    return 0;
  }
  if (strcmp(name, "lstm_cluster_write_through") == 0) {
    h->lstm_cluster_wt = value != 0;
    return 0;
  }
  if (strcmp(name, "lstm_cluster_rows") == 0) {
    if (value < 0) return fail(h, "lstm_cluster_rows must be >= 0");
    h->lstm_cluster_rows = value;
    return 0;
  }
  if (strcmp(name, "lstm_small_rows") == 0) {
    if (value < 0) return fail(h, "lstm_small_rows must be >= 0");
    h->lstm_small_rows = value;
    return 0;
  }
  if (strcmp(name, "lstm_x_table") == 0) {
    if (value < 0 || value > 2) return fail(h, "lstm_x_table must be 0 (off), 1 (batches with B * T >= vocab_size) or 2 (always)");
    h->lstm_x_table = value;
    return 0;
  }
  if (strcmp(name, "lstm_x_table_mb") == 0) {
    if (value < 0) return fail(h, "lstm_x_table_mb must be >= 0");
    h->lstm_x_table_mb = value;
    return 0;
  }
  return fail(h, "unknown option '%s'", name);
}

int sse_l2_normalize_dev(sse_handle *h, const float *x_dev, float *out_dev, int64_t rows, int32_t cols, void *stream) {
  if (!h) return 1;
  std::lock_guard<std::mutex> lk(h->mu);
  HIPCHECK(h, hipSetDevice(h->cfg.device));
  HIPCHECK(h, launch_l2_normalize(x_dev, out_dev, rows, cols, (hipStream_t)stream));
  return 0;
}

int sse_index_set_dev(sse_handle *h, const float *rows_dev, int64_t N, int32_t S, int64_t id_base, void *stream) {
  if (!h) return 1;
  std::lock_guard<std::mutex> lk(h->mu);
  HIPCHECK(h, hipSetDevice(h->cfg.device));
  if (h->idx64) {
    HIPCHECK(h, hipFree(h->idx64));
    h->idx64 = nullptr;
// ... 1110 lines not shown
```

sequence-semantic-embedding_amd/csrc/sse_kernels.h:

```cpp
#pragma once
#include <hip/hip_runtime.h>
#include <stdint.h>

typedef float f32x4 __attribute__((ext_vector_type(4)));
typedef float f32x16 __attribute__((ext_vector_type(16)));

__host__ __device__ static inline int frag32_off(int r_in_tile, int k_in_group) {
  return ((((k_in_group >> 2) << 5) + r_in_tile) << 2) + (k_in_group & 3);
}

__device__ static inline int mfma_row(int reg, int lane) { return (reg & 3) + 8 * (reg >> 2) + 4 * (lane >> 5); }

static inline int round_up(int x, int m) { return (x + m - 1) / m * m; }

typedef unsigned int sse_u32x4 __attribute__((ext_vector_type(4)));
__host__ __device__ static inline unsigned short sse_bf16_rne(float f) {
  unsigned u;
  __builtin_memcpy(&u, &f, 4);
  u += 0x7FFFu + ((u >> 16) & 1u);
  return (unsigned short)(u >> 16);
}
__host__ __device__ static inline float sse_bf16_f32(unsigned short h) {
  const unsigned u = (unsigned)h << 16;
  float f;
// ... 117 lines not shown

struct LstmX3Args {
  const int32_t *ids;
  const unsigned short *emb16;
  const unsigned short *Wx3;
  const float *Mp;
  float *out;
  int32_t *err;
  int32_t B, T, V, KGX, H, S, NTS, normalize;
  const int32_t *row_map = nullptr;
  const float *pad_h = nullptr, *pad_c = nullptr;
  float *rec_h = nullptr, *rec_c = nullptr;
  float *tape_g = nullptr, *tape_a = nullptr, *h_last = nullptr;
  int32_t NT32 = 0;
  int32_t tiles_elsewhere = 0;
};
int lstm_x3_kgx(int E);
size_t lstm_x3_weight_elems(int E, int Hp);
size_t lstm_x3_emb_elems(int64_t V, int E);
hipError_t launch_pack_lstm_x3(const float *K, const float *b, const float *emb , int64_t V, int E, int H,
                               int Hp, unsigned short *Wx3, unsigned short *emb16 ,
                               int natural_k , hipStream_t stream);
hipError_t launch_lstm_fwd_x3(const LstmX3Args &a, hipStream_t stream);

struct LstmPersistArgs {
  const int32_t *ids;
  const float *emb;
  const float *Waug;
  const float *M;
  float *out;
  int32_t *err;
  int32_t B, T, V, E, H, S, normalize;
  const float *pad_h = nullptr, *pad_c = nullptr;
  int32_t pad_stride = 0;
  unsigned long long *hx = nullptr;
  unsigned long long *rawx = nullptr;
  uint32_t epoch = 0;
  int32_t NWG = 0;
  int32_t map_mode = 0;
  int32_t write_through = 0;
  int32_t plain_launch = 0;
};
int lstm_persist_nwg(int E, int H, int S);
int lstm_persist_max_rows();
int lstm_persist_max_steps();
size_t lstm_persist_hx_words(int H);
size_t lstm_persist_raw_words(int S);
hipError_t launch_lstm_persist(const LstmPersistArgs &a, hipStream_t stream);
void lstm_note_coop_refused();
long long lstm_coop_refused();

struct LstmClusterArgs {
  const int32_t *ids;
  const float *emb;
  const float *Wc;
  const float *Mp;
  float *out;
  int32_t *err;
  int32_t B, T, V, E, Ep, KGx, KGh, H, Hp, S, NTS, normalize;
  const float *pad_h = nullptr, *pad_c = nullptr;
  int32_t pad_stride = 0;
  unsigned long long *hx = nullptr;
  unsigned long long *sx = nullptr;
  uint32_t epoch = 0;
  int32_t NCL = 0;
  int32_t write_through = 0;
  int32_t plain_launch = 0;
  int32_t drop_wg = 0;
};
int lstm_cluster_ok(int E, int H, int S);
int lstm_cluster_max_rows();
size_t lstm_cluster_weight_floats(int E, int H);
size_t lstm_cluster_hx_words(int H);
size_t lstm_cluster_sx_words();
hipError_t launch_pack_lstm_cluster(const float *K, const float *b, int E, int H, float *Wc, hipStream_t stream);
hipError_t launch_lstm_cluster(const LstmClusterArgs &a, hipStream_t stream);

struct ScoreArgs {
  const float *idxp;
  const float *qp;
  float *part_scores;
  int32_t *part_ids;
  float *part_bnd;
  int64_t N;
  int32_t Q, KG, NT, QT, NSPLIT, KC;
  int32_t NQ = 4;
  int32_t thr_off = 0;
  const int32_t *q_count = nullptr;
  int32_t BF = 0;
  int32_t COLLECT = 0;
  const float *col_thr = nullptr;
  const int32_t *col_slot = nullptr;
  int32_t *col_cnt = nullptr;
  int32_t *col_buf = nullptr;
  int32_t col_cap = 0;
  float *lane_max = nullptr;
  int32_t dbg = 0;
  const float *q_rows = nullptr;
  int32_t S = 0;
  const int32_t *uncert = nullptr;
};
hipError_t launch_score_topk(const ScoreArgs &a, hipStream_t stream);
hipError_t launch_lane_max_threshold(const float *q, const float *lane_max, int Q, int S, int NV, float eps, float *col_thr,
                                     int32_t *col_slot, hipStream_t st);
#define SSE_MAX_INDEX_DIM 1024
int score_pick_nq(int Q, int S, int with_bf16);
size_t score_lds_bytes(int NQ, int KG, int BF, int COLLECT);
hipError_t launch_pack_rows_bf16(const float *rows, int64_t R, int C, void *out, hipStream_t stream);
hipError_t launch_count_uncert(const int32_t *cert, int Q, unsigned long long *count, hipStream_t st);
hipError_t launch_compact_uncert(const float *q, const int32_t *cert, int Q, int S, int32_t *qmap, int32_t *count, float *qc,
                                 hipStream_t st);
hipError_t launch_frag32_to_bf16(const float *idxp, int64_t NT, int KG, void *out, hipStream_t stream);
hipError_t launch_frag32_to_split_bf16(const float *idxp, int64_t NT, int KG, void *out, hipStream_t stream);

#define SSE_COLLECT_CAP 4096
#define SSE_MAX_SELECT_K 1024

struct RescoreArgs {
  const float *q;
  const float *idx32;
  const double *idx64;
  const float *part_scores;
  const int32_t *part_ids;
  const float *part_bnd;
  double *out_scores;
  int64_t *out_ids;
  int32_t *cert;
  int64_t id_base, N;
  int32_t Q, S, NC, k;
  float eps;
  const int32_t *qmap = nullptr, *q_count = nullptr;
  float *col_thr = nullptr;
  float eps32 = 0.0f;
  int32_t *col_slot = nullptr, *col_cnt = nullptr;
  double *host_scores = nullptr;
  int64_t *host_ids = nullptr;
  int32_t *host_cert = nullptr, *host_flag = nullptr, *host_err = nullptr;
  const int32_t *err_in = nullptr;
  int32_t seq = 0;
  const float *idx_rm = nullptr;
  int32_t *uncert = nullptr, *uncert_clear = nullptr;
};
hipError_t launch_rescore(const RescoreArgs &a, hipStream_t stream);

struct SmallIndexArgs {
  const float *q_rows;
  const float *idxp;
  float *part_scores;
  int32_t *part_ids;
  float *part_bnd;
  int64_t N;
  int32_t Q, S, KG, NT;
  const void *idx_x3 = nullptr;
};
bool score_small_index_applies(int Q, int KG, int64_t NT);
hipError_t launch_score_small_index(const SmallIndexArgs &a, hipStream_t stream);

hipError_t launch_assign_slots(const int32_t *cert, int Q, int slots, int32_t *col_slot, int32_t *counter, hipStream_t st);
hipError_t launch_kth_bound(const float *q, const float *part_scores, const int32_t *part_ids, int Q, int S, int NC, int k,
                            float eps, float *col_thr, int32_t *col_slot, hipStream_t st);
struct SelectArgs {
  const float *q;
  const float *idx32;
  const double *idx64;
  const int32_t *col_slot, *col_cnt, *col_buf;
  int32_t col_cap;
  double *out_scores;
  int64_t *out_ids;
  int32_t *cert;
  int64_t id_base;
  int32_t Q, S, k;
  unsigned long long *served = nullptr;
  const int32_t *uncert = nullptr;
  int32_t grid_cap = 0;
};
hipError_t launch_select_topk(const SelectArgs &a, hipStream_t st);

hipError_t launch_merge_topk(const double *in_s, const int64_t *in_i, int64_t stride, int P, int Q, int k, double *out_s,
                             int64_t *out_i, hipStream_t stream);

hipError_t launch_pack_rows(const float *rows, int64_t R, int C, float *out, hipStream_t stream);
hipError_t launch_pack_rows_norm(const float *rows, int64_t R, int C, float *out, float *norm_bits, hipStream_t stream);
hipError_t launch_f64_to_f32(const double *in, float *out, int64_t n, hipStream_t stream);
hipError_t launch_l2_normalize(const float *x, float *out, int64_t rows, int cols, hipStream_t stream);

hipError_t launch_pack_lstm(const float *K, const float *b, int E, int H, int Ep, int Hp, int UB, float *Wp,
                            hipStream_t stream);
enum { PACK_JOB_PAD_ROWS = 1, PACK_JOB_LSTM = 2, PACK_JOB_KN = 3, PACK_JOB_KT = 4 };
struct PackJob {
  int32_t type;
  const float *a, *b;
  float *out;
  int64_t total;
  int32_t i0, i1, i2, i3;
};
#define SSE_MAX_PACK_JOBS 12
struct PackJobs {
  PackJob job[SSE_MAX_PACK_JOBS];
  int32_t n = 0;
};
void pack_job_pad_rows(PackJobs &js, const float *in, int64_t R, int C, int Cp, int one_col, float *out);
void pack_job_lstm(PackJobs &js, const float *K, const float *b, int E, int H, int Ep, int Hp, float *Wp);
void pack_job_kn(PackJobs &js, const float *X, int K, int N, int KGp, float *out);
void pack_job_kT(PackJobs &js, const float *K, int row0, int nrows, int RT, int H, int Hp, float *out);
hipError_t launch_pack_multi(const PackJobs &js, hipStream_t stream);
hipError_t launch_pack_kn(const float *X, int K, int N, int KGp, float *out, hipStream_t stream);
hipError_t launch_pad_rows(const float *in, int64_t R, int C, int Cp, int one_col, float *out, hipStream_t stream);
#define SSE_PAD_SORT_MAX_T 8192
size_t pad_sort_zeroed_words();
size_t pad_sort_work_words(int B, int T);
hipError_t launch_pad_sort(const int32_t *ids, int B, int T, int32_t *zeroed, int32_t *work, int32_t *order, int32_t *stat_pinned,
                           int32_t seq, bool scatter, hipStream_t stream);
hipError_t launch_row_norm2_max(const float *x, int64_t rows, int cols, float *out_bits, hipStream_t stream);
hipError_t launch_fill(float *p, int64_t n, float v, hipStream_t stream);
hipError_t launch_exact_topk(const float *q, const float *idxp, const double *idx64, const int32_t *cert,
                             double *out_scores, int64_t *out_ids, int64_t id_base, int64_t N, int Q, int S,
                             int k, hipStream_t stream, unsigned long long *served = nullptr, const int32_t *uncert = nullptr,
                             int grid_cap = 0);

size_t cnn_bf16_packed_weight_elems(int Ep);
size_t cnn_bf16_lds_bytes(int T, int Ep, int train);
hipError_t launch_cnn_bf16_pack(const float *emb, int64_t V, int E, int Ep, unsigned short *emb_bf16, const float *const W[4],
                                unsigned short *Wc, hipStream_t stream);
hipError_t launch_cnn_fwd_bf16(const int32_t *ids, const unsigned short *emb_bf16, const unsigned short *Wc, const float *bias,
                               float *featp, int32_t *err, int B, int T, int V, int Ep, float *feat_rm, int32_t *pos,
                               hipStream_t stream);
hipError_t launch_cnn_proj(const float *featp, const float *Mp, float *out, int B, int S, int normalize, hipStream_t stream);
size_t cnn_proj_x3_elems(int S);
hipError_t launch_pack_cnn_proj_x3(const float *Mv, int S, unsigned short *Mx3, hipStream_t stream);
hipError_t launch_cnn_proj_x3(const float *featp, const unsigned short *Mx3, float *out, int B, int S, int normalize, hipStream_t stream);
size_t cnn_lds_bytes(int T, int Ep, int train);
size_t cnn_packed_weight_floats(int Ep);
hipError_t launch_pack_conv(const float *const W[4], int E, int Ep, float *out, hipStream_t stream);
hipError_t launch_cnn_fwd(const int32_t *ids, const float *emb, const float *Wc, const float *bias, const float *Mp,
                          float *featp, float *out, int32_t *err, int B, int T, int V, int Ep, int S, int normalize,
                          float *feat_rm , int32_t *pos ,
                          hipStream_t stream);
```

Before: 7.608 million seqs/s.

## Fuse float64 rescore tail into small-index scoring kernel

Moves the exact float64 rescore of the top candidates into the small-index score/select kernel, so each wave rescores its queries right after selection instead of the work running as a separate rescore launch. This is meant to remove a kernel launch and the global round trip of partial scores and ids for the 571-target case. The change adds a launch bound of two blocks per CU, more register pressure from the float64 path, and a larger kernel argument struct. It is on by default only for the SCORE_ALL phase without a host mirror.

```diff
diff --git a/sequence-semantic-embedding_amd/csrc/score_topk.hip b/sequence-semantic-embedding_amd/csrc/score_topk.hip
--- a/sequence-semantic-embedding_amd/csrc/score_topk.hip
+++ b/sequence-semantic-embedding_amd/csrc/score_topk.hip
@@ -847,308 +847,6 @@
   return hipGetLastError();
 }
 
-__device__ __forceinline__ int si_key(float f) {
-  const int i = __float_as_int(f);
-  return i >= 0 ? i : (i ^ 0x7FFFFFFF);
-}
-__device__ __forceinline__ float si_val(int k) { return __int_as_float(k >= 0 ? k : (k ^ 0x7FFFFFFF)); }
-template <int CTRL, int ROWMASK>
-__device__ __forceinline__ float dpp_f(float x) {
-  return __int_as_float(__builtin_amdgcn_update_dpp(__float_as_int(x), __float_as_int(x), CTRL, ROWMASK, 0xF, false));
-}
-__device__ __forceinline__ float wave_max_f(float x) {
-  x = fmaxf(x, dpp_f<0x128, 0xF>(x));
-  x = fmaxf(x, dpp_f<0x124, 0xF>(x));
-  x = fmaxf(x, dpp_f<0x122, 0xF>(x));
-  x = fmaxf(x, dpp_f<0x121, 0xF>(x));
-  x = fmaxf(x, dpp_f<0x142, 0xA>(x));
-  x = fmaxf(x, dpp_f<0x143, 0xC>(x));
-  return __int_as_float(__builtin_amdgcn_readlane(__float_as_int(x), 63));
-}
-template <int JMAX>
-#ifdef SSE_SCORE_CLOCK
-#define SI_CLK_PARAMS , long long (&ck_)[8], long long &ck_t
-#define SI_CLK_ARGS , ck_, ck_t
-#else
-#define SI_CLK_PARAMS
-#define SI_CLK_ARGS
-#endif
-__device__ __forceinline__ void si_select4(const SmallIndexArgs &a, const float *sc, int NP, int NT, int qt, int q0, int lane SI_CLK_PARAMS) {
-  constexpr int QW = 4;
-  const int J = (NT * 32 + 63) / 64;
-  float v[QW][JMAX];
-#pragma unroll
-  for (int j = 0; j < JMAX; ++j) {
-    const int row = lane + 64 * j;
-#pragma unroll
-    for (int c = 0; c < QW; ++c) v[c][j] = (j < J && row < NT * 32) ? sc[(q0 + c) * NP + row] : NEG_INF;
-  }
-  int lok[QW], hik[QW];
-  float lm[QW];
-  bool done[QW];
-#pragma unroll
-  for (int c = 0; c < QW; ++c) {
-    float m = NEG_INF;
-#pragma unroll
-    for (int j = 0; j < JMAX; ++j) m = fmaxf(m, v[c][j]);
-    lm[c] = m;
-    lok[c] = si_key(-wave_max_f(-m));
-    hik[c] = si_key(wave_max_f(m)) + 1;
-    done[c] = false;
-  }
-  SC_CLK(5)
-  for (;;) {
-    bool all_done = true;
-#pragma unroll
-    for (int c = 0; c < QW; ++c) {
-      const unsigned width = (unsigned)hik[c] - (unsigned)lok[c];
-      const int mid = lok[c] + (int)(width >> 1);
-      const int cnt = __popcll(__ballot(lm[c] >= si_val(mid)));
-      const bool open = !done[c] && width > 1u;
-      const bool ge = cnt >= SC_KC;
-      lok[c] = (open && ge) ? mid : lok[c];
-      hik[c] = (open && !ge) ? mid : hik[c];
-      done[c] = !open || (ge && cnt <= 24);
-      all_done = all_done && done[c];
-    }
-    if (all_done) break;
-  }
-  SC_CLK(6)
-#pragma unroll
-  for (int c = 0; c < QW; ++c) {
-    const int query = qt * 32 + q0 + c;
-    if (query < a.Q) {
-      const float T = si_val(lok[c]);
-      float cs = NEG_INF;
-      int cr = -1, base = 0;
-#pragma unroll
-      for (int j = 0; j < JMAX; ++j) {
-        const bool take = (j < J) & (v[c][j] >= T) & (v[c][j] > NEG_INF);
-        const unsigned long long mask = __ballot(take);
-        const int n = __popcll(mask);
-        const int slot = base + (int)__builtin_amdgcn_mbcnt_hi((unsigned)(mask >> 32), __builtin_amdgcn_mbcnt_lo((unsigned)mask, 0u));
-        const int dst = (take && slot < 63) ? slot : 63;
-        const int gs = __builtin_amdgcn_ds_permute(dst * 4, __float_as_int(v[c][j]));
-        const int gr = __builtin_amdgcn_ds_permute(dst * 4, lane + 64 * j);
-        const bool recv = (lane >= base) & (lane < base + n) & (lane < 63);
-        cs = recv ? __int_as_float(gs) : cs;
-        cr = recv ? gr : cr;
-        base += n;
-      }
-      const int nw = base < 63 ? base : 63;
-      int rank = 0;
-      for (int l = 0; l < nw; ++l) {
-        const float os = __int_as_float(__builtin_amdgcn_readlane(__float_as_int(cs), l));
-        const int orow = __builtin_amdgcn_readlane(cr, l);
-        rank += ((os > cs) | ((os == cs) & (orow < cr))) ? 1 : 0;
-      }
-      const bool mine = lane < nw;
-      if (mine && rank < SC_KC) {
-        a.part_scores[(size_t)query * SC_KC + rank] = cs;
-        a.part_ids[(size_t)query * SC_KC + rank] = cr;
-      }
-      if (lane >= nw && lane < SC_KC) {
-        a.part_scores[(size_t)query * SC_KC + lane] = NEG_INF;
-        a.part_ids[(size_t)query * SC_KC + lane] = -1;
-      }
-      const unsigned long long m16 = __ballot(mine && rank == SC_KC - 1);
-      const float last = m16 ? __int_as_float(__builtin_amdgcn_readlane(__float_as_int(cs), __ffsll((long long)m16) - 1)) : NEG_INF;
-      if (lane == 0) a.part_bnd[query] = (base > 63) ? __builtin_inff() : last;
-    }
-  }
-}
-
-template <int KGC>
-__global__ __launch_bounds__(256) void score_small_index_kernel(SmallIndexArgs a) {
-  extern __shared__ __attribute__((aligned(16))) float si_sc[];
-  const int tid = threadIdx.x, lane = tid & 63, w = __builtin_amdgcn_readfirstlane(tid >> 6);
-  const int NT = a.NT, NP = NT * 32 + 1;
-  const int qt = blockIdx.x;
-  float *sc = si_sc;
-  SC_CLK_DECL
-  f32x4 b[KGC];
-  {
-    const int row = qt * 32 + (lane & 31), kb = (lane >> 5) * 4;
-    const float *src = a.q_rows + (size_t)(row < a.Q ? row : 0) * a.S + kb;
-    const bool vec = (a.S & 3) == 0 && (reinterpret_cast<uintptr_t>(a.q_rows) & 15) == 0 && KGC * 8 <= a.S;
-#pragma unroll
-    for (int kg = 0; kg < KGC; ++kg) {
-      f32x4 v = {0, 0, 0, 0};
-      if (vec) {
-        v = *reinterpret_cast<const f32x4 *>(src + kg * 8);
-      } else {
-#pragma unroll
-        for (int e = 0; e < 4; ++e)
-          if (kg * 8 + kb + e < a.S) v[e] = src[kg * 8 + e];
-      }
-      if (row >= a.Q) v = f32x4{0, 0, 0, 0};
-      b[kg] = v;
-    }
-  }
-  SC_CLK(0)
-  for (int t = w; t < NT; t += 4) {
-    const f32x4 *ap = reinterpret_cast<const f32x4 *>(a.idxp) + (size_t)t * KGC * 64 + lane;
-    f32x16 acc = {0, 0, 0, 0, 0, 0, 0, 0, 0, 0, 0, 0, 0, 0, 0, 0};
-    f32x4 ar[4];
-#pragma unroll
-    for (int d = 0; d < 4; ++d) ar[d] = ap[(d < KGC ? d : 0) * 64];
-#pragma unroll
-    for (int kg = 0; kg < KGC; ++kg) {
-      __builtin_amdgcn_sched_barrier(0);
-#pragma unroll
-      for (int e = 0; e < 4; ++e) acc = __builtin_amdgcn_mfma_f32_32x32x2f32(ar[kg & 3][e], b[kg][e], acc, 0, 0, 0);
-      __builtin_amdgcn_sched_barrier(0);
-      ar[kg & 3] = ap[(kg + 4 < KGC ? kg + 4 : kg) * 64];
-    }
-    const int rb = t * 32 + 4 * (lane >> 5);
-    float *col = sc + (lane & 31) * NP;
-#pragma unroll
-    for (int r = 0; r < 16; ++r) {
-      const int row = rb + (r & 3) + 8 * (r >> 2);
-      col[row] = (row < a.N) ? acc[r] : NEG_INF;
-    }
-  }
-  SC_CLK(1)
-  __syncthreads();
-  SC_CLK(2)
-  if (NT * 32 <= 640) {
-    si_select4<10>(a, sc, NP, NT, qt, w * 8, lane SI_CLK_ARGS);
-    SC_CLK(3)
-    si_select4<10>(a, sc, NP, NT, qt, w * 8 + 4, lane SI_CLK_ARGS);
-    SC_CLK(4)
-#ifdef SSE_SCORE_CLOCK
-    if (blockIdx.x == gridDim.x / 2 && lane == 0)
-      for (int i = 0; i < 8; ++i) g_score_clk[w * 8 + i] = ck_[i];
-#endif
-  } else {
-    si_select4<16>(a, sc, NP, NT, qt, w * 8, lane SI_CLK_ARGS);
-    si_select4<16>(a, sc, NP, NT, qt, w * 8 + 4, lane SI_CLK_ARGS);
-  }
-}
-template <int KB>
-__global__ __launch_bounds__(256) void score_small_index_x3_kernel(SmallIndexArgs a) {
-  extern __shared__ __attribute__((aligned(16))) float si_sc[];
-  const int tid = threadIdx.x, lane = tid & 63, w = __builtin_amdgcn_readfirstlane(tid >> 6);
-  const int NT = a.NT, NP = NT * 32 + 1;
-  const int qt = blockIdx.x;
-  float *sc = si_sc;
-  SC_CLK_DECL
-  sse_u32x4 bh[KB], bl[KB];
-  {
-    const int row = qt * 32 + (lane & 31), kb0 = (lane >> 5) * 8;
-    const float *src = a.q_rows + (size_t)(row < a.Q ? row : 0) * a.S + kb0;
-    const bool vec = (a.S & 3) == 0 && (reinterpret_cast<uintptr_t>(a.q_rows) & 15) == 0 && KB * 16 <= a.S;
-#pragma unroll
-    for (int kb = 0; kb < KB; ++kb) {
-      float v[8] = {0, 0, 0, 0, 0, 0, 0, 0};
-      if (vec) {
-        const f32x4 v0 = *reinterpret_cast<const f32x4 *>(src + kb * 16), v1 = *reinterpret_cast<const f32x4 *>(src + kb * 16 + 4);
-#pragma unroll
-        for (int e = 0; e < 4; ++e) {
-          v[e] = v0[e];
-          v[4 + e] = v1[e];
-        }
-      } else {
-#pragma unroll
-        for (int e = 0; e < 8; ++e)
-          if (kb * 16 + kb0 + e < a.S) v[e] = src[kb * 16 + e];
-      }
-      if (row >= a.Q) {
-#pragma unroll
-        for (int e = 0; e < 8; ++e) v[e] = 0.0f;
-      }
-      sse_split8(v, bh[kb], bl[kb]);
-    }
-  }
-  SC_CLK(0)
-  {
-    constexpr int D = KB < 4 ? KB : 4;
-    static_assert(KB % D == 0, "the ring index must be static");
-    const sse_u32x4 *img = reinterpret_cast<const sse_u32x4 *>(a.idx_x3) + lane;
-    const sse_u32x4 *ap = img + (size_t)(w < NT ? w : 0) * KB * 128;
-    sse_u32x4 ah[D], al[D];
-#pragma unroll
-    for (int d = 0; d < D; ++d) {
-      ah[d] = ap[d * 128];
-      al[d] = ap[d * 128 + 64];
-    }
-    for (int t = w; t < NT; t += 4) {
-      const sse_u32x4 *apn = img + (size_t)(t + 4 < NT ? t + 4 : t) * KB * 128;
-      f32x16 acc = {0, 0, 0, 0, 0, 0, 0, 0, 0, 0, 0, 0, 0, 0, 0, 0};
-#pragma unroll
-      for (int kb = 0; kb < KB; ++kb) {
-        __builtin_amdgcn_sched_barrier(0);
-        const bf16x8_t xh = __builtin_bit_cast(bf16x8_t, ah[kb % D]), xl = __builtin_bit_cast(bf16x8_t, al[kb % D]);
-        const bf16x8_t yh = __builtin_bit_cast(bf16x8_t, bh[kb]), yl = __builtin_bit_cast(bf16x8_t, bl[kb]);
-        acc = __builtin_amdgcn_mfma_f32_32x32x16_bf16(xh, yh, acc, 0, 0, 0);
-        acc = __builtin_amdgcn_mfma_f32_32x32x16_bf16(xh, yl, acc, 0, 0, 0);
-        acc = __builtin_amdgcn_mfma_f32_32x32x16_bf16(xl, yh, acc, 0, 0, 0);
-        __builtin_amdgcn_sched_barrier(0);
-        const sse_u32x4 *nx = (kb + D < KB) ? ap + (kb + D) * 128 : apn + (kb + D - KB) * 128;
-        ah[kb % D] = nx[0];
-        al[kb % D] = nx[64];
-      }
-      const int rb = t * 32 + 4 * (lane >> 5);
-      float *col = sc + (lane & 31) * NP;
-#pragma unroll
-      for (int r = 0; r < 16; ++r) {
-        const int row = rb + (r & 3) + 8 * (r >> 2);
-        col[row] = (row < a.N) ? acc[r] : NEG_INF;
-      }
-      ap = apn;
-    }
-  }
-  SC_CLK(1)
-  __syncthreads();
-  SC_CLK(2)
-  if (NT * 32 <= 640) {
-    si_select4<10>(a, sc, NP, NT, qt, w * 8, lane SI_CLK_ARGS);
-    SC_CLK(3)
-    si_select4<10>(a, sc, NP, NT, qt, w * 8 + 4, lane SI_CLK_ARGS);
-    SC_CLK(4)
-#ifdef SSE_SCORE_CLOCK
-    if (blockIdx.x == gridDim.x / 2 && lane == 0)
-      for (int i = 0; i < 8; ++i) g_score_clk[w * 8 + i] = ck_[i];
-#endif
-  } else {
-    si_select4<16>(a, sc, NP, NT, qt, w * 8, lane SI_CLK_ARGS);
-    si_select4<16>(a, sc, NP, NT, qt, w * 8 + 4, lane SI_CLK_ARGS);
-  }
-}
-bool score_small_index_applies(int Q, int KG, int64_t NT) {
-  return Q >= 1024 && (KG == 32 || KG == 8 || KG == 7) && NT * 32 <= 1024 && (size_t)32 * (NT * 32 + 1) * sizeof(float) <= (size_t)144 * 1024;
-}
-hipError_t launch_score_small_index(const SmallIndexArgs &a, hipStream_t stream) {
-  if (!score_small_index_applies(a.Q, a.KG, a.NT)) return hipErrorInvalidValue;
-  const size_t lds = (size_t)32 * (a.NT * 32 + 1) * sizeof(float);
-  const dim3 grid((a.Q + 31) / 32), block(256);
-  auto go = [&](auto kernel) -> hipError_t {
-    hipError_t e = hipFuncSetAttribute(reinterpret_cast<const void *>(kernel), hipFuncAttributeMaxDynamicSharedMemorySize, (int)lds);
-    if (e != hipSuccess) return e;
-    hipLaunchKernelGGL(kernel, grid, block, lds, stream, a);
-    return hipGetLastError();
-  };
-  if (a.idx_x3 && a.KG != 32) return go(score_small_index_x3_kernel<4>);
-  if (a.KG == 8) return go(score_small_index_kernel<8>);
-  if (a.KG == 7) return go(score_small_index_kernel<7>);
-  const hipError_t e32 = a.idx_x3 ? go(score_small_index_x3_kernel<16>) : go(score_small_index_kernel<32>);
-  if (e32 != hipSuccess) return e32;
-#ifdef SSE_SCORE_CLOCK
-  if (a.Q >= 8192) {
-    static int n = 0;
-    if (n++ % 8 == 3) {
-      long long v[64];
-      (void)hipStreamSynchronize(stream);
-      (void)hipMemcpyFromSymbol(v, HIP_SYMBOL(g_score_clk), sizeof v);
-      for (int w = 0; w < 4; w += 3)
-        fprintf(stderr, "[small index clock Q=%d NT=%d] wave %d cycles: query fragments %lld | scores (MFMA + LDS stores) %lld | barrier %lld | selection: loads + bounds %lld | bisection %lld | winners + rank + stores %lld (both batches)\n",
-                a.Q, a.NT, w, v[w * 8 + 0], v[w * 8 + 1], v[w * 8 + 2], v[w * 8 + 5], v[w * 8 + 6], v[w * 8 + 3] + v[w * 8 + 4]);
-    }
-  }
-#endif
-  return hipGetLastError();
-}
-
 hipError_t launch_score_topk(const ScoreArgs &a_in, hipStream_t stream) {
   ScoreArgs a = a_in;
 #ifdef SSE_SCORE_MEASURE
@@ -1242,6 +940,23 @@
   return lane;
 }
 template <int NB>
+__device__ __forceinline__ double wave_packed_reduce(double (&acc)[NB], int lane) {
+  int m = 32;
+#pragma unroll
+  for (int cnt = NB; cnt > 1; cnt >>= 1, m >>= 1) {
+    const bool up = (lane & m) != 0;
+#pragma unroll
+    for (int i = 0; i < cnt / 2; ++i) {
+      const double send = up ? acc[i] : acc[i + cnt / 2];
+      const double keep = up ? acc[i + cnt / 2] : acc[i];
+      acc[i] = keep + __shfl_xor(send, m);
+    }
+  }
+#pragma unroll
+  for (; m > 0; m >>= 1) acc[0] += __shfl_xor(acc[0], m);
+  return acc[0];
+}
+template <int NB>
 __device__ __forceinline__ double wave_exact_dot_packed(const float *qrow, const float *idxp, const double *idx64, const int64_t (&n)[NB],
                                                         int S, int KG, int lane, const float *idx_rm = nullptr) {
   static_assert(NB == 2 || NB == 4 || NB == 8, "power of two");
@@ -1273,20 +988,7 @@
         }
     }
   }
-  int m = 32;
-#pragma unroll
-  for (int cnt = NB; cnt > 1; cnt >>= 1, m >>= 1) {
-    const bool up = (lane & m) != 0;
-#pragma unroll
-    for (int i = 0; i < cnt / 2; ++i) {
-      const double send = up ? acc[i] : acc[i + cnt / 2];
-      const double keep = up ? acc[i + cnt / 2] : acc[i];
-      acc[i] = keep + __shfl_xor(send, m);
-    }
-  }
-#pragma unroll
-  for (; m > 0; m >>= 1) acc[0] += __shfl_xor(acc[0], m);
-  return acc[0];
+  return wave_packed_reduce<NB>(acc, lane);
 }
 
 __device__ __forceinline__ bool before(double sa, int64_t ia, double sb, int64_t ib) {
@@ -1480,10 +1182,189 @@
 #ifndef RS_NB
 #define RS_NB 4
 #endif
+#define RS_PRE 16
 __device__ __forceinline__ double readlane_f64(double v, int l) {
   const long long b = __double_as_longlong(v);
   const int lo = __builtin_amdgcn_readlane((int)b, l), hi = __builtin_amdgcn_readlane((int)(b >> 32), l);
   return __longlong_as_double(((long long)hi << 32) | (unsigned int)lo);
+}
+template <bool PRE>
+struct RsSmallWin {
+  int idm, nwin;
+  float qnorm, eps_q, mmax;
+  double exm;
+  bool pre;
+  f32x4 qv;
+  f32x4 v[PRE ? 16 : 1];
+};
+template <int CTRL>
+__device__ __forceinline__ double quad_dpp_f64(double x) {
+  const long long b = __double_as_longlong(x);
+  const int lo = __builtin_amdgcn_update_dpp((int)b, (int)b, CTRL, 0xF, 0xF, false);
+  const int hi = __builtin_amdgcn_update_dpp((int)(b >> 32), (int)(b >> 32), CTRL, 0xF, 0xF, false);
+  return __longlong_as_double(((long long)hi << 32) | (unsigned int)lo);
+}
+__device__ __forceinline__ float wave_query_norm(const float *qrow, int S, int lane) {
+  double qn = 0.0;
+  for (int d = lane; d < S; d += 64) qn += (double)qrow[d] * qrow[d];
+#pragma unroll
+  for (int o = 32; o > 0; o >>= 1) qn += __shfl_xor(qn, o);
+  return (float)sqrt(qn);
+}
+__device__ __forceinline__ void wave_query_norm4(const float (&x)[4][4], int S, int lane, float (&out)[4]) {
+  double acc[4] = {0.0, 0.0, 0.0, 0.0};
+#pragma unroll
+  for (int t = 0; t < 4; ++t)
+    if (lane + 64 * t < S) {
+#pragma unroll
+      for (int c = 0; c < 4; ++c) acc[c] += (double)x[c][t] * x[c][t];
+    }
+  const double tot = wave_packed_reduce<4>(acc, lane);
+#pragma unroll
+  for (int c = 0; c < 4; ++c) out[c] = (float)sqrt(readlane_f64(tot, packed_lane_of_value<4>(c)));
+}
+template <bool PRE, bool RANKED>
+__device__ __forceinline__ void rescore_small_begin(const RescoreArgs &a, const float *qrow, int KG, int lane, int id, float sc,
+                                                    int rank_in, float qnorm, float mmax, RsSmallWin<PRE> &w) {
+  w.qnorm = qnorm;
+  w.eps_q = a.eps * qnorm;
+  w.mmax = mmax;
+  int rank = rank_in;
+  unsigned u = __float_as_uint(sc);
+  u = (u & 0x80000000u) ? ~u : (u | 0x80000000u);
+  const unsigned long long key = (id < 0) ? 0ull : (((unsigned long long)u << 32) | (unsigned long long)(0xFFFFFFFFu - (unsigned)id));
+  if (!RANKED) {
+    const int key_lo = (int)(unsigned)key, key_hi = (int)(unsigned)(key >> 32);
+    rank = 0;
+    for (int j = 0; j < a.NC; ++j) {
+      const unsigned long long kj = ((unsigned long long)(unsigned)__builtin_amdgcn_readlane(key_hi, j) << 32) |
+                                    (unsigned long long)(unsigned)__builtin_amdgcn_readlane(key_lo, j);
+      rank += (kj > key) ? 1 : 0;
+    }
+  }
+  const unsigned long long kmask = __ballot(key != 0ull && rank == a.k - 1);
+  const float kth = kmask ? __int_as_float(__builtin_amdgcn_readlane(__float_as_int(sc), __ffsll((long long)kmask) - 1)) : NEG_INF;
+  const bool in_win = (id >= 0) && (sc >= kth - 2.0f * w.eps_q);
+  const unsigned long long wmask = __ballot(in_win);
+  w.nwin = __popcll(wmask);
+  const int mi = __popcll(wmask & ((1ull << lane) - 1ull));
+  w.idm = __builtin_amdgcn_ds_permute((in_win ? mi : 63) * 4, id);
+  w.exm = -__builtin_inf();
+  w.pre = false;
+  if (PRE) {
+    w.pre = !a.idx64 && KG * 2 <= 64 && w.nwin <= RS_PRE;
+    if (w.pre) {
+      const int s = lane & 3;
+      const int64_t n = __shfl(w.idm, lane >> 2);
+      const bool valid = (lane >> 2) < w.nwin;
+      const bool qvec = (a.S & 3) == 0 && (reinterpret_cast<uintptr_t>(qrow) & 15) == 0;
+      w.qv = f32x4{0, 0, 0, 0};
+      if (4 * lane < a.S) {
+        if (qvec && 4 * lane + 4 <= a.S) {
+          w.qv = *reinterpret_cast<const f32x4 *>(qrow + 4 * lane);
+        } else {
+#pragma unroll
+          for (int e = 0; e < 4; ++e)
+            if (4 * lane + e < a.S) w.qv[e] = qrow[4 * lane + e];
+        }
+      }
+      const float *base = a.idx_rm ? a.idx_rm + (size_t)n * a.S + s * 4
+                                   : a.idx32 + (size_t)(n >> 5) * KG * 256 + (s >> 1) * 256 + ((s & 1) * 32 + (int)(n & 31)) * 4;
+#pragma unroll
+      for (int i = 0; i < 16; ++i) w.v[i] = f32x4{0, 0, 0, 0};
+      const int ni = valid ? (a.S - 4 * s + 15) >> 4 : 0;
+      if (a.idx_rm) {
+#pragma unroll
+        for (int i = 0; i < 16; ++i)
+          if (i < ni) w.v[i] = *reinterpret_cast<const f32x4 *>(base + i * 16);
+      } else {
+#pragma unroll
+        for (int i = 0; i < 16; ++i)
+          if (i < ni) {
+            w.v[i] = *reinterpret_cast<const f32x4 *>(base + i * 512);
+#pragma unroll
+            for (int e = 0; e < 4; ++e)
+              if (4 * (s + 4 * i) + e >= a.S) w.v[i][e] = 0.0f;
+          }
+      }
+    }
+  }
+}
+template <bool PRE>
+__device__ __forceinline__ void rescore_small_dots(const RescoreArgs &a, const float *qrow, int KG, int lane, RsSmallWin<PRE> &w) {
+  if (PRE && w.pre) {
+    const int s = lane & 3;
+    double leaf[PRE ? 16 : 1];
+#pragma unroll
+    for (int i = 0; i < (PRE ? 16 : 0); ++i) {
+      leaf[i] = 0.0;
+      if (4 * i < KG * 2) {
+        const int j = s + 4 * i;
+        float qj[4];
+#pragma unroll
+        for (int e = 0; e < 4; ++e) qj[e] = __int_as_float(__builtin_amdgcn_ds_bpermute(j * 4, __float_as_int(w.qv[e])));
+#pragma unroll
+        for (int e = 0; e < 4; ++e) leaf[i] += (double)qj[e] * (double)w.v[i][e];
+        if (i & 1) __builtin_amdgcn_sched_barrier(0);
+      }
+    }
+    if (PRE) {
+#pragma unroll
+      for (int h = 8; h > 0; h >>= 1)
+#pragma unroll
+        for (int i = 0; i < h; ++i) leaf[i] += leaf[i + h];
+      double t = leaf[0];
+      t += quad_dpp_f64<0x4E>(t);
+      t += quad_dpp_f64<0xB1>(t);
+      const double got = __shfl(t, (lane * 4) & 63);
+      if (lane < w.nwin) w.exm = got;
+    }
+    return;
+  }
+  for (int m0 = 0; m0 < w.nwin; m0 += RS_NB) {
+    int64_t n[RS_NB];
+#pragma unroll
+    for (int c = 0; c < RS_NB; ++c) n[c] = __builtin_amdgcn_readlane(w.idm, (m0 + c < w.nwin) ? m0 + c : 0);
+    const double tot = wave_exact_dot_packed<RS_NB>(qrow, a.idx32, a.idx64, n, a.S, KG, lane, a.idx_rm);
+    const int want = lane - m0;
+    const double got = __shfl(tot, packed_lane_of_value<RS_NB>(want & (RS_NB - 1)));
+    if (want >= 0 && want < RS_NB && lane < w.nwin) w.exm = got;
+  }
+}
+template <bool PRE>
+__device__ __forceinline__ void rescore_small_finish(const RescoreArgs &a, int qo, int lane, const RsSmallWin<PRE> &w) {
+  const double exm = w.exm;
+  const int idm = w.idm, nwin = w.nwin;
+  int r2 = 0;
+  for (int j = 0; j < nwin; ++j)
+    r2 += before(readlane_f64(exm, j), (int64_t)__builtin_amdgcn_readlane(idm, j), exm, (int64_t)idm) ? 1 : 0;
+  const bool member = lane < nwin;
+  if (member && r2 < a.k) {
+    a.out_scores[(size_t)qo * a.k + r2] = exm;
+    a.out_ids[(size_t)qo * a.k + r2] = a.id_base + idm;
+    if (a.host_flag) {
+      a.host_scores[(size_t)qo * a.k + r2] = exm;
+      a.host_ids[(size_t)qo * a.k + r2] = a.id_base + idm;
+    }
+  }
+  const unsigned long long tmask = __ballot(member && r2 == a.k - 1);
+  const double theta = tmask ? readlane_f64(exm, __ffsll((long long)tmask) - 1) : -__builtin_inf();
+  if (a.host_flag) __threadfence_system();
+  if (lane == 0) {
+    const bool ok = (nwin >= a.k) && ((double)w.mmax + (double)w.eps_q < theta);
+    a.cert[qo] = ok ? 1 : 0;
+    if (!ok && a.uncert) atomicAdd(a.uncert, 1);
+    if (a.col_thr) a.col_thr[qo] = ok ? __builtin_inff() : __double2float_rd(theta - (double)(a.eps32 * w.qnorm));
+    if (a.col_slot) {
+      a.col_slot[qo] = ok ? -1 : qo;
+      a.col_cnt[qo] = 0;
+    }
+    if (a.host_flag) {
+      a.host_cert[qo] = ok ? 1 : 0;
+      if (qo == 0 && a.host_err) *a.host_err = a.err_in ? *a.err_in : 0;
+      __hip_atomic_store(a.host_flag + qo, a.seq, __ATOMIC_RELEASE, __HIP_MEMORY_SCOPE_SYSTEM);
+    }
+  }
 }
 __global__ __launch_bounds__(256) void rescore_small_kernel(RescoreArgs a) {
   const int lane = threadIdx.x & 63;
@@ -1504,82 +1385,23 @@
   const int id = have ? a.part_ids[(size_t)q * a.NC + lane] : -1;
   const float sc = have ? a.part_scores[(size_t)q * a.NC + lane] : NEG_INF;
   const float bnd = (lane < a.NC / SC_KC) ? a.part_bnd[(size_t)q * (a.NC / SC_KC) + lane] : NEG_INF;
-  double qn = 0.0;
-  for (int d = lane; d < a.S; d += 64) qn += (double)qrow[d] * qrow[d];
-#pragma unroll
-  for (int o = 32; o > 0; o >>= 1) qn += __shfl_xor(qn, o);
-  const float qnorm = (float)sqrt(qn);
-  const float eps_q = a.eps * qnorm;
+  const float qnorm = wave_query_norm(qrow, a.S, lane);
   RS_CLK(0)
-
-  unsigned u = __float_as_uint(sc);
-  u = (u & 0x80000000u) ? ~u : (u | 0x80000000u);
-  const unsigned long long key = (id < 0) ? 0ull : (((unsigned long long)u << 32) | (unsigned long long)(0xFFFFFFFFu - (unsigned)id));
-  const int key_lo = (int)(unsigned)key, key_hi = (int)(unsigned)(key >> 32);
-  int rank = 0;
-  for (int j = 0; j < a.NC; ++j) {
-    const unsigned long long kj = ((unsigned long long)(unsigned)__builtin_amdgcn_readlane(key_hi, j) << 32) |
-                                  (unsigned long long)(unsigned)__builtin_amdgcn_readlane(key_lo, j);
-    rank += (kj > key) ? 1 : 0;
-  }
-  const unsigned long long kmask = __ballot(key != 0ull && rank == a.k - 1);
-  const float kth = kmask ? __int_as_float(__builtin_amdgcn_readlane(__float_as_int(sc), __ffsll((long long)kmask) - 1)) : NEG_INF;
-  const bool in_win = (id >= 0) && (sc >= kth - 2.0f * eps_q);
   float mmax = NEG_INF;
   for (int j = 0; j < a.NC / SC_KC; ++j) mmax = fmaxf(mmax, __int_as_float(__builtin_amdgcn_readlane(__float_as_int(bnd), j)));
-  const unsigned long long wmask = __ballot(in_win);
-  const int nwin = __popcll(wmask);
-  const int mi = __popcll(wmask & ((1ull << lane) - 1ull));
-  const int idm = __builtin_amdgcn_ds_permute((in_win ? mi : 63) * 4, id);
+  RsSmallWin<false> w;
+  rescore_small_begin<false, false>(a, qrow, KG, lane, id, sc, 0, qnorm, mmax, w);
   RS_CLK(1)
-  double exm = -__builtin_inf();
-  for (int m0 = 0; m0 < nwin; m0 += RS_NB) {
-    int64_t n[RS_NB];
-#pragma unroll
-    for (int c = 0; c < RS_NB; ++c) n[c] = __builtin_amdgcn_readlane(idm, (m0 + c < nwin) ? m0 + c : 0);
-    const double tot = wave_exact_dot_packed<RS_NB>(qrow, a.idx32, a.idx64, n, a.S, KG, lane, a.idx_rm);
-    const int want = lane - m0;
-    const double got = __shfl(tot, packed_lane_of_value<RS_NB>(want & (RS_NB - 1)));
-    if (want >= 0 && want < RS_NB && lane < nwin) exm = got;
-  }
+  rescore_small_dots<false>(a, qrow, KG, lane, w);
   RS_CLK(2)
-  int r2 = 0;
-  for (int j = 0; j < nwin; ++j)
-    r2 += before(readlane_f64(exm, j), (int64_t)__builtin_amdgcn_readlane(idm, j), exm, (int64_t)idm) ? 1 : 0;
-  const bool member = lane < nwin;
-  if (member && r2 < a.k) {
-    a.out_scores[(size_t)qo * a.k + r2] = exm;
-    a.out_ids[(size_t)qo * a.k + r2] = a.id_base + idm;
-    if (a.host_flag) {
-      a.host_scores[(size_t)qo * a.k + r2] = exm;
-      a.host_ids[(size_t)qo * a.k + r2] = a.id_base + idm;
-    }
-  }
-  const unsigned long long tmask = __ballot(member && r2 == a.k - 1);
-  const double theta = tmask ? readlane_f64(exm, __ffsll((long long)tmask) - 1) : -__builtin_inf();
-  if (a.host_flag) __threadfence_system();
+  rescore_small_finish<false>(a, qo, lane, w);
   RS_CLK(3)
 #ifdef SSE_SCORE_CLOCK
   if (q == a.Q / 2 && lane == 0) {
-    rk_[4] = nwin;
+    rk_[4] = w.nwin;
     for (int i = 0; i < 6; ++i) g_score_clk[i] = rk_[i];
   }
 #endif
-  if (lane == 0) {
-    const bool ok = (nwin >= a.k) && ((double)mmax + (double)eps_q < theta);
-    a.cert[qo] = ok ? 1 : 0;
-    if (!ok && a.uncert) atomicAdd(a.uncert, 1);
-    if (a.col_thr) a.col_thr[qo] = ok ? __builtin_inff() : __double2float_rd(theta - (double)(a.eps32 * qnorm));
-    if (a.col_slot) {
-      a.col_slot[qo] = ok ? -1 : qo;
-      a.col_cnt[qo] = 0;
-    }
-    if (a.host_flag) {
-      a.host_cert[qo] = ok ? 1 : 0;
-      if (qo == 0 && a.host_err) *a.host_err = a.err_in ? *a.err_in : 0;
-      __hip_atomic_store(a.host_flag + qo, a.seq, __ATOMIC_RELEASE, __HIP_MEMORY_SCOPE_SYSTEM);
-    }
-  }
 }
 
 hipError_t launch_rescore(const RescoreArgs &a, hipStream_t stream) {
@@ -1601,6 +1423,384 @@
     return hipGetLastError();
   }
   hipLaunchKernelGGL(rescore_kernel, dim3(a.Q), dim3(RS_THREADS), (size_t)a.NC * sizeof(unsigned long long), stream, a);
+  return hipGetLastError();
+}
+
+__device__ __forceinline__ int si_key(float f) {
+  const int i = __float_as_int(f);
+  return i >= 0 ? i : (i ^ 0x7FFFFFFF);
+}
+__device__ __forceinline__ float si_val(int k) { return __int_as_float(k >= 0 ? k : (k ^ 0x7FFFFFFF)); }
+template <int CTRL, int ROWMASK>
+__device__ __forceinline__ float dpp_f(float x) {
+  return __int_as_float(__builtin_amdgcn_update_dpp(__float_as_int(x), __float_as_int(x), CTRL, ROWMASK, 0xF, false));
+}
+__device__ __forceinline__ float wave_max_f(float x) {
+  x = fmaxf(x, dpp_f<0x128, 0xF>(x));
+  x = fmaxf(x, dpp_f<0x124, 0xF>(x));
+  x = fmaxf(x, dpp_f<0x122, 0xF>(x));
+  x = fmaxf(x, dpp_f<0x121, 0xF>(x));
+  x = fmaxf(x, dpp_f<0x142, 0xA>(x));
+  x = fmaxf(x, dpp_f<0x143, 0xC>(x));
+  return __int_as_float(__builtin_amdgcn_readlane(__float_as_int(x), 63));
+}
+template <int JMAX, bool FUSED>
+#ifdef SSE_SCORE_CLOCK
+#define SI_CLK_PARAMS , long long (&ck_)[8], long long &ck_t
+#define SI_CLK_ARGS , ck_, ck_t
+#else
+#define SI_CLK_PARAMS
+#define SI_CLK_ARGS
+#endif
+__device__ __forceinline__ void si_select4(const SmallIndexArgs &a, const float *sc, int NP, int NT, int qt, int q0, int lane SI_CLK_PARAMS) {
+  constexpr int QW = 4;
+  const int J = (NT * 32 + 63) / 64;
+  float qnorm[QW], qx[QW][4];
+  if (FUSED) {
+#pragma unroll
+    for (int c = 0; c < QW; ++c) {
+      const int query = qt * 32 + q0 + c;
+      const float *qr = a.rs.q + (size_t)(query < a.Q ? query : 0) * a.S;
+#pragma unroll
+      for (int t = 0; t < 4; ++t) qx[c][t] = (lane + 64 * t < a.S) ? qr[lane + 64 * t] : 0.0f;
+    }
+  }
+  float v[QW][JMAX];
+#pragma unroll
+  for (int j = 0; j < JMAX; ++j) {
+    const int row = lane + 64 * j;
+#pragma unroll
+    for (int c = 0; c < QW; ++c) v[c][j] = (j < J && row < NT * 32) ? sc[(q0 + c) * NP + row] : NEG_INF;
+  }
+  int lok[QW], hik[QW];
+  float lm[QW];
+  bool done[QW];
+#pragma unroll
+  for (int c = 0; c < QW; ++c) {
+    float m = NEG_INF;
+#pragma unroll
+    for (int j = 0; j < JMAX; ++j) m = fmaxf(m, v[c][j]);
+    lm[c] = m;
+    lok[c] = si_key(-wave_max_f(-m));
+    hik[c] = si_key(wave_max_f(m)) + 1;
+    done[c] = false;
+  }
+  SC_CLK(5)
+  for (;;) {
+    bool all_done = true;
+#pragma unroll
+    for (int c = 0; c < QW; ++c) {
+      const unsigned width = (unsigned)hik[c] - (unsigned)lok[c];
+      const int mid = lok[c] + (int)(width >> 1);
+      const int cnt = __popcll(__ballot(lm[c] >= si_val(mid)));
+      const bool open = !done[c] && width > 1u;
+      const bool ge = cnt >= SC_KC;
+      lok[c] = (open && ge) ? mid : lok[c];
+      hik[c] = (open && !ge) ? mid : hik[c];
+      done[c] = !open || (ge && cnt <= 24);
+      all_done = all_done && done[c];
+    }
+    if (all_done) break;
+  }
+  SC_CLK(6)
+  if (FUSED) wave_query_norm4(qx, a.S, lane, qnorm);
+  float wsc[QW], wbnd[QW];
+  int wid[QW], wrank[QW];
+  RsSmallWin<FUSED> w;
+  auto tail_begin = [&](int c) {
+    const int query = qt * 32 + q0 + c;
+    rescore_small_begin<FUSED, true>(a.rs, a.rs.q + (size_t)query * a.S, a.KG, lane, wid[c], wsc[c], wrank[c], qnorm[c], wbnd[c], w);
+  };
+  auto tail_end = [&](int c) {
+    const int query = qt * 32 + q0 + c;
+    rescore_small_dots<FUSED>(a.rs, a.rs.q + (size_t)query * a.S, a.KG, lane, w);
+    rescore_small_finish<FUSED>(a.rs, query, lane, w);
+  };
+  {
+    float cs[QW];
+    int cr[QW], base[QW];
+#pragma unroll
+    for (int c = 0; c < QW; ++c) {
+      cs[c] = NEG_INF;
+      cr[c] = -1;
+      base[c] = 0;
+    }
+#pragma unroll
+    for (int j = 0; j < JMAX; ++j) {
+      int gs[QW], gr[QW], n[QW];
+#pragma unroll
+      for (int c = 0; c < QW; ++c) {
+        const float T = si_val(lok[c]);
+        const bool take = (j < J) & (v[c][j] >= T) & (v[c][j] > NEG_INF);
+        const unsigned long long mask = __ballot(take);
+        n[c] = __popcll(mask);
+        const int slot = base[c] + (int)__builtin_amdgcn_mbcnt_hi((unsigned)(mask >> 32), __builtin_amdgcn_mbcnt_lo((unsigned)mask, 0u));
+        const int dst = (take && slot < 63) ? slot : 63;
+        gs[c] = __builtin_amdgcn_ds_permute(dst * 4, __float_as_int(v[c][j]));
+        gr[c] = __builtin_amdgcn_ds_permute(dst * 4, lane + 64 * j);
+      }
+#pragma unroll
+      for (int c = 0; c < QW; ++c) {
+        const bool recv = (lane >= base[c]) & (lane < base[c] + n[c]) & (lane < 63);
+        cs[c] = recv ? __int_as_float(gs[c]) : cs[c];
+        cr[c] = recv ? gr[c] : cr[c];
+        base[c] += n[c];
+      }
+    }
+    int nw[QW], nwmax = 0;
+#pragma unroll
+    for (int c = 0; c < QW; ++c) {
+      nw[c] = base[c] < 63 ? base[c] : 63;
+      nwmax = nw[c] > nwmax ? nw[c] : nwmax;
+      wrank[c] = 0;
+    }
+    for (int l = 0; l < nwmax; ++l) {
+#pragma unroll
+      for (int c = 0; c < QW; ++c) {
+        const float os = __int_as_float(__builtin_amdgcn_readlane(__float_as_int(cs[c]), l));
+        const int orow = __builtin_amdgcn_readlane(cr[c], l);
+        wrank[c] += ((os > cs[c]) | ((os == cs[c]) & (orow < cr[c]))) ? 1 : 0;
+      }
+    }
+#pragma unroll
+    for (int c = 0; c < QW; ++c) {
+      const bool mine = lane < nw[c];
+      const unsigned long long m16 = __ballot(mine && wrank[c] == SC_KC - 1);
+      const float last = m16 ? __int_as_float(__builtin_amdgcn_readlane(__float_as_int(cs[c]), __ffsll((long long)m16) - 1)) : NEG_INF;
+      wbnd[c] = (base[c] > 63) ? __builtin_inff() : last;
+      wsc[c] = (mine && wrank[c] < SC_KC) ? cs[c] : NEG_INF;
+      wid[c] = (mine && wrank[c] < SC_KC) ? cr[c] : -1;
+    }
+  }
+  if (!FUSED) {
+#pragma unroll
+    for (int c = 0; c < QW; ++c) {
+      const int query = qt * 32 + q0 + c;
+      if (query < a.Q) {
+        if (wid[c] >= 0) {
+          a.part_scores[(size_t)query * SC_KC + wrank[c]] = wsc[c];
+          a.part_ids[(size_t)query * SC_KC + wrank[c]] = wid[c];
+        }
+        const int nc = __popcll(__ballot(wid[c] >= 0));
+        if (lane >= nc && lane < SC_KC) {
+          a.part_scores[(size_t)query * SC_KC + lane] = NEG_INF;
+          a.part_ids[(size_t)query * SC_KC + lane] = -1;
+        }
+        if (lane == 0) a.part_bnd[query] = wbnd[c];
+      }
+    }
+    return;
+  }
+  const int live = a.Q - (qt * 32 + q0);
+  SC_CLK(3)
+#pragma unroll
+  for (int c = 0; c < QW; ++c)
+    if (c < live) {
+      tail_begin(c);
+      tail_end(c);
+    }
+  SC_CLK(7)
+}
+
+template <int KGC, bool FUSED>
+__global__ __launch_bounds__(256, 2) void score_small_index_kernel(SmallIndexArgs a) {
+  extern __shared__ __attribute__((aligned(16))) float si_sc[];
+  const int tid = threadIdx.x, lane = tid & 63, w = __builtin_amdgcn_readfirstlane(tid >> 6);
+  const int NT = a.NT, NP = NT * 32 + 1;
+  const int qt = blockIdx.x;
+  float *sc = si_sc;
+  if (FUSED && a.rs.uncert_clear && blockIdx.x == 0 && tid == 0) *a.rs.uncert_clear = 0;
+  SC_CLK_DECL
+  f32x4 b[KGC];
+  {
+    const int row = qt * 32 + (lane & 31), kb = (lane >> 5) * 4;
+    const float *src = a.q_rows + (size_t)(row < a.Q ? row : 0) * a.S + kb;
+    const bool vec = (a.S & 3) == 0 && (reinterpret_cast<uintptr_t>(a.q_rows) & 15) == 0 && KGC * 8 <= a.S;
+#pragma unroll
+    for (int kg = 0; kg < KGC; ++kg) {
+      f32x4 v = {0, 0, 0, 0};
+      if (vec) {
+        v = *reinterpret_cast<const f32x4 *>(src + kg * 8);
+      } else {
+#pragma unroll
+        for (int e = 0; e < 4; ++e)
+          if (kg * 8 + kb + e < a.S) v[e] = src[kg * 8 + e];
+      }
+      if (row >= a.Q) v = f32x4{0, 0, 0, 0};
+      b[kg] = v;
+    }
+  }
+  SC_CLK(0)
+  for (int t = w; t < NT; t += 4) {
+    const f32x4 *ap = reinterpret_cast<const f32x4 *>(a.idxp) + (size_t)t * KGC * 64 + lane;
+    f32x16 acc = {0, 0, 0, 0, 0, 0, 0, 0, 0, 0, 0, 0, 0, 0, 0, 0};
+    f32x4 ar[4];
+#pragma unroll
+    for (int d = 0; d < 4; ++d) ar[d] = ap[(d < KGC ? d : 0) * 64];
+#pragma unroll
+    for (int kg = 0; kg < KGC; ++kg) {
+      __builtin_amdgcn_sched_barrier(0);
+#pragma unroll
+      for (int e = 0; e < 4; ++e) acc = __builtin_amdgcn_mfma_f32_32x32x2f32(ar[kg & 3][e], b[kg][e], acc, 0, 0, 0);
+      __builtin_amdgcn_sched_barrier(0);
+      ar[kg & 3] = ap[(kg + 4 < KGC ? kg + 4 : kg) * 64];
+    }
+    const int rb = t * 32 + 4 * (lane >> 5);
+    float *col = sc + (lane & 31) * NP;
+#pragma unroll
+    for (int r = 0; r < 16; ++r) {
+      const int row = rb + (r & 3) + 8 * (r >> 2);
+      col[row] = (row < a.N) ? acc[r] : NEG_INF;
+    }
+  }
+  SC_CLK(1)
+  __syncthreads();
+  SC_CLK(2)
+  if (NT * 32 <= 640) {
+    si_select4<10, FUSED>(a, sc, NP, NT, qt, w * 8, lane SI_CLK_ARGS);
+    SC_CLK(3)
+    si_select4<10, FUSED>(a, sc, NP, NT, qt, w * 8 + 4, lane SI_CLK_ARGS);
+    SC_CLK(4)
+#ifdef SSE_SCORE_CLOCK
+    if (blockIdx.x == gridDim.x / 2 && lane == 0)
+      for (int i = 0; i < 8; ++i) g_score_clk[w * 8 + i] = ck_[i];
+#endif
+  } else {
+    si_select4<16, FUSED>(a, sc, NP, NT, qt, w * 8, lane SI_CLK_ARGS);
+    si_select4<16, FUSED>(a, sc, NP, NT, qt, w * 8 + 4, lane SI_CLK_ARGS);
+  }
+}
+template <int KB, bool FUSED>
+__global__ __launch_bounds__(256, 2) void score_small_index_x3_kernel(SmallIndexArgs a) {
+  extern __shared__ __attribute__((aligned(16))) float si_sc[];
+  const int tid = threadIdx.x, lane = tid & 63, w = __builtin_amdgcn_readfirstlane(tid >> 6);
+  const int NT = a.NT, NP = NT * 32 + 1;
+  const int qt = blockIdx.x;
+  float *sc = si_sc;
+  if (FUSED && a.rs.uncert_clear && blockIdx.x == 0 && tid == 0) *a.rs.uncert_clear = 0;
+  SC_CLK_DECL
+  sse_u32x4 bh[KB], bl[KB];
+  {
+    const int row = qt * 32 + (lane & 31), kb0 = (lane >> 5) * 8;
+    const float *src = a.q_rows + (size_t)(row < a.Q ? row : 0) * a.S + kb0;
+    const bool vec = (a.S & 3) == 0 && (reinterpret_cast<uintptr_t>(a.q_rows) & 15) == 0 && KB * 16 <= a.S;
+#pragma unroll
+    for (int kb = 0; kb < KB; ++kb) {
+      float v[8] = {0, 0, 0, 0, 0, 0, 0, 0};
+      if (vec) {
+        const f32x4 v0 = *reinterpret_cast<const f32x4 *>(src + kb * 16), v1 = *reinterpret_cast<const f32x4 *>(src + kb * 16 + 4);
+#pragma unroll
+        for (int e = 0; e < 4; ++e) {
+          v[e] = v0[e];
+          v[4 + e] = v1[e];
+        }
+      } else {
+#pragma unroll
+        for (int e = 0; e < 8; ++e)
+          if (kb * 16 + kb0 + e < a.S) v[e] = src[kb * 16 + e];
+      }
+      if (row >= a.Q) {
+#pragma unroll
+        for (int e = 0; e < 8; ++e) v[e] = 0.0f;
+      }
+      sse_split8(v, bh[kb], bl[kb]);
+    }
+  }
+  SC_CLK(0)
+  {
+    constexpr int D = KB < 4 ? KB : 4;
+    static_assert(KB % D == 0, "the ring index must be static");
+    const sse_u32x4 *img = reinterpret_cast<const sse_u32x4 *>(a.idx_x3) + lane;
+    const sse_u32x4 *ap = img + (size_t)(w < NT ? w : 0) * KB * 128;
+    sse_u32x4 ah[D], al[D];
+#pragma unroll
+    for (int d = 0; d < D; ++d) {
+      ah[d] = ap[d * 128];
+      al[d] = ap[d * 128 + 64];
+    }
+    for (int t = w; t < NT; t += 4) {
+      const sse_u32x4 *apn = img + (size_t)(t + 4 < NT ? t + 4 : t) * KB * 128;
+      f32x16 acc = {0, 0, 0, 0, 0, 0, 0, 0, 0, 0, 0, 0, 0, 0, 0, 0};
+#pragma unroll
+      for (int kb = 0; kb < KB; ++kb) {
+        __builtin_amdgcn_sched_barrier(0);
+        const bf16x8_t xh = __builtin_bit_cast(bf16x8_t, ah[kb % D]), xl = __builtin_bit_cast(bf16x8_t, al[kb % D]);
+        const bf16x8_t yh = __builtin_bit_cast(bf16x8_t, bh[kb]), yl = __builtin_bit_cast(bf16x8_t, bl[kb]);
+        acc = __builtin_amdgcn_mfma_f32_32x32x16_bf16(xh, yh, acc, 0, 0, 0);
+        acc = __builtin_amdgcn_mfma_f32_32x32x16_bf16(xh, yl, acc, 0, 0, 0);
+        acc = __builtin_amdgcn_mfma_f32_32x32x16_bf16(xl, yh, acc, 0, 0, 0);
+        __builtin_amdgcn_sched_barrier(0);
+        const sse_u32x4 *nx = (kb + D < KB) ? ap + (kb + D) * 128 : apn + (kb + D - KB) * 128;
+        ah[kb % D] = nx[0];
+        al[kb % D] = nx[64];
+      }
+      const int rb = t * 32 + 4 * (lane >> 5);
+      float *col = sc + (lane & 31) * NP;
+#pragma unroll
+      for (int r = 0; r < 16; ++r) {
+        const int row = rb + (r & 3) + 8 * (r >> 2);
+        col[row] = (row < a.N) ? acc[r] : NEG_INF;
+      }
+      ap = apn;
+    }
+  }
+  SC_CLK(1)
+  __syncthreads();
+  SC_CLK(2)
+  if (NT * 32 <= 640) {
+    si_select4<10, FUSED>(a, sc, NP, NT, qt, w * 8, lane SI_CLK_ARGS);
+    SC_CLK(3)
+    si_select4<10, FUSED>(a, sc, NP, NT, qt, w * 8 + 4, lane SI_CLK_ARGS);
+    SC_CLK(4)
+#ifdef SSE_SCORE_CLOCK
+    if (blockIdx.x == gridDim.x / 2 && lane == 0)
+      for (int i = 0; i < 8; ++i) g_score_clk[w * 8 + i] = ck_[i];
+#endif
+  } else {
+    si_select4<16, FUSED>(a, sc, NP, NT, qt, w * 8, lane SI_CLK_ARGS);
+    si_select4<16, FUSED>(a, sc, NP, NT, qt, w * 8 + 4, lane SI_CLK_ARGS);
+  }
+}
+bool score_small_index_applies(int Q, int KG, int64_t NT) {
+  return Q >= 1024 && (KG == 32 || KG == 8 || KG == 7) && NT * 32 <= 1024 && (size_t)32 * (NT * 32 + 1) * sizeof(float) <= (size_t)144 * 1024;
+}
+hipError_t launch_score_small_index(const SmallIndexArgs &a, hipStream_t stream) {
+  if (!score_small_index_applies(a.Q, a.KG, a.NT)) return hipErrorInvalidValue;
+  const size_t lds = (size_t)32 * (a.NT * 32 + 1) * sizeof(float);
+  const dim3 grid((a.Q + 31) / 32), block(256);
+  auto go = [&](auto kernel) -> hipError_t {
+    hipError_t e = hipFuncSetAttribute(reinterpret_cast<const void *>(kernel), hipFuncAttributeMaxDynamicSharedMemorySize, (int)lds);
+    if (e != hipSuccess) return e;
+    hipLaunchKernelGGL(kernel, grid, block, lds, stream, a);
+    return hipGetLastError();
+  };
+  hipError_t e32;
+  if (a.fused) {
+    if (a.rs.NC != SC_KC || a.rs.qmap || a.rs.q_count || a.rs.host_flag || a.rs.q != a.q_rows || a.rs.S != a.S || a.rs.Q != a.Q) return hipErrorInvalidValue;
+    if (a.idx_x3 && a.KG != 32) return go(score_small_index_x3_kernel<4, true>);
+    if (a.KG == 8) return go(score_small_index_kernel<8, true>);
+    if (a.KG == 7) return go(score_small_index_kernel<7, true>);
+    e32 = a.idx_x3 ? go(score_small_index_x3_kernel<16, true>) : go(score_small_index_kernel<32, true>);
+  } else {
+    if (a.idx_x3 && a.KG != 32) return go(score_small_index_x3_kernel<4, false>);
+    if (a.KG == 8) return go(score_small_index_kernel<8, false>);
+    if (a.KG == 7) return go(score_small_index_kernel<7, false>);
+    e32 = a.idx_x3 ? go(score_small_index_x3_kernel<16, false>) : go(score_small_index_kernel<32, false>);
+  }
+  if (e32 != hipSuccess) return e32;
+#ifdef SSE_SCORE_CLOCK
+  if (a.Q >= 8192) {
+    static int n = 0;
+    if (n++ % 8 == 3) {
+      long long v[64];
+      (void)hipStreamSynchronize(stream);
+      (void)hipMemcpyFromSymbol(v, HIP_SYMBOL(g_score_clk), sizeof v);
+      for (int w = 0; w < 4; w += 3)
+        fprintf(stderr, "[small index clock Q=%d NT=%d] wave %d cycles: query fragments %lld | scores (MFMA + LDS stores) %lld | barrier %lld | selection: loads + bounds %lld | bisection %lld | winners + rank + stores %lld | fused float64 tail %lld (both batches)\n",
+                a.Q, a.NT, w, v[w * 8 + 0], v[w * 8 + 1], v[w * 8 + 2], v[w * 8 + 5], v[w * 8 + 6], v[w * 8 + 3] + v[w * 8 + 4], v[w * 8 + 7]);
+    }
+  }
+#endif
   return hipGetLastError();
 }
 
diff --git a/sequence-semantic-embedding_amd/csrc/sse_api.hip b/sequence-semantic-embedding_amd/csrc/sse_api.hip
--- a/sequence-semantic-embedding_amd/csrc/sse_api.hip
+++ b/sequence-semantic-embedding_amd/csrc/sse_api.hip
@@ -144,6 +144,7 @@
   int lstm_x_table_mb = 256;
   int64_t x_table_builds = 0;
   bool score_small_index = true;
+  bool score_small_fused = true;
   bool score_small_x3 = true;
   bool score_bf16 = true;
   void *idxp16 = nullptr;
@@ -1190,15 +1191,6 @@
   a.NSPLIT = nsplit;
   a.KC = 16;
   a.NQ = NQ;
-  if (first) {
-    if (small_idx) {
-      SmallIndexArgs si{q, h->idxp, a.part_scores, a.part_ids, a.part_bnd, h->idx_N, Q, S, KG, (int)NT};
-      if (small_x3) si.idx_x3 = h->idx_x3.p;
-      HIPCHECK(h, launch_score_small_index(si, st));
-    } else {
-      HIPCHECK(h, launch_score_topk(a, st));
-    }
-  }
   RescoreArgs r;
   r.q = q;
   r.idx32 = h->idxp;
@@ -1233,7 +1225,21 @@
   if (bf) r.eps += (float)(1.02 * (1.0 / 256.0 + 1.0 / 262144.0) * h->idx_norm_max);
   if (small_x3)
     r.eps = (float)(((1.0 + 1.0 / 64.0) / 32768.0 + 2.0 * (3 * S + 2) * 5.97e-8 * (1.0 + 1.0 / 32.0)) * h->idx_norm_max);
+  const bool small_fused = small_idx && h->score_small_fused && !mirror && phase == SCORE_ALL;
   if (first) {
+    if (small_idx) {
+      SmallIndexArgs si{q, h->idxp, a.part_scores, a.part_ids, a.part_bnd, h->idx_N, Q, S, KG, (int)NT};
+      if (small_x3) si.idx_x3 = h->idx_x3.p;
+      if (small_fused) {
+        si.fused = 1;
+        si.rs = r;
+      }
+      HIPCHECK(h, launch_score_small_index(si, st));
+    } else {
+      HIPCHECK(h, launch_score_topk(a, st));
+    }
+  }
+  if (first && !small_fused) {
     RescoreArgs rf = r;
     if (mirror) {
       rf.host_scores = mirror->scores;
@@ -1741,6 +1747,10 @@
   }
   if (strcmp(name, "score_small_x3") == 0) {
     h->score_small_x3 = value != 0;
+    return 0;
+  }
+  if (strcmp(name, "score_small_fused") == 0) {
+    h->score_small_fused = value != 0;
     return 0;
   }
   if (strcmp(name, "score_bf16") == 0) {
diff --git a/sequence-semantic-embedding_amd/csrc/sse_kernels.h b/sequence-semantic-embedding_amd/csrc/sse_kernels.h
--- a/sequence-semantic-embedding_amd/csrc/sse_kernels.h
+++ b/sequence-semantic-embedding_amd/csrc/sse_kernels.h
@@ -293,6 +293,8 @@
   int64_t N;
   int32_t Q, S, KG, NT;
   const void *idx_x3 = nullptr;
+  int32_t fused = 0;
+  RescoreArgs rs;
 };
 bool score_small_index_applies(int Q, int KG, int64_t NT);
 hipError_t launch_score_small_index(const SmallIndexArgs &a, hipStream_t stream);
```

Result: no change. 7.635 million seqs/s, median of 6 (+0.4%).
